# andreaskoepf/faster-rcnn.torch

Hardware: AMD Instinct MI355X
Metric: images/sec (vgg_small 800x450 fwd+bwd) (higher is better)
Workload: dtype f32 (conv / Linear(13824,1024) operands as 2 x fp16 split planes: 22 significand bits, 3 MFMA partial products; fp32 accumulate)

## Files before the change

faster-rcnn.torch_amd/_lib.py:

```python
import ctypes as C
import os

_HERE = os.path.dirname(os.path.abspath(__file__))
SO_PATH = os.environ.get("FRCNN_LIB_PATH") or os.path.join(_HERE, "libfrcnn_hip.so")

KC_NAMES = ["conv_igemm_k3", "conv_igemm_other", "conv_wgrad_k3", "conv_wgrad_other", "gemm", "elemwise",
            "roi", "rpn", "nms", "optim", "image", "conv_x3", "conv_wgradx"]


class FrcnnError(RuntimeError):
    pass


class ModelDesc(C.Structure):
    _fields_ = [
        ("nblocks", C.c_int),
        ("filters", C.c_int * 8), ("ksize", C.c_int * 8), ("pad", C.c_int * 8), ("conv_steps", C.c_int * 8),
        ("dropout", C.c_float * 8),
        ("nheads", C.c_int),
        ("head_k", C.c_int * 8), ("head_n", C.c_int * 8), ("head_input", C.c_int * 8),
        ("ncls", C.c_int),
        ("cls_n", C.c_int * 8), ("cls_bn", C.c_int * 8),
        ("cls_dropout", C.c_float * 8),
        ("class_count", C.c_int),
        ("kh", C.c_int), ("kw", C.c_int),
    ]


vp = C.c_void_p
_SIGS = {
    "frcnn_version": ([], C.c_int),
    "frcnn_set_option": ([C.c_char_p, C.c_int], C.c_int),
    "frcnn_get_option": ([C.c_char_p, C.POINTER(C.c_int)], C.c_int),
    "frcnn_last_error": ([], C.c_char_p),
    "frcnn_device_count": ([C.POINTER(C.c_int)], C.c_int),
    "frcnn_set_device": ([C.c_int], C.c_int),
    "frcnn_device_name": ([C.c_char_p, C.c_int], C.c_int),
    "frcnn_malloc": ([C.POINTER(vp), C.c_size_t], C.c_int),
    "frcnn_free": ([vp], C.c_int),
    "frcnn_host_alloc": ([C.POINTER(vp), C.c_size_t], C.c_int),
    "frcnn_host_free": ([vp], C.c_int),
    "frcnn_memcpy_h2d": ([vp, vp, C.c_size_t, vp], C.c_int),
    "frcnn_memcpy_d2h": ([vp, vp, C.c_size_t, vp], C.c_int),
    "frcnn_memcpy_d2d": ([vp, vp, C.c_size_t, vp], C.c_int),
    "frcnn_stream_sync": ([vp], C.c_int),
    "frcnn_zero": ([vp, C.c_size_t, vp], C.c_int),
    "frcnn_scale": ([vp, C.c_longlong, C.c_float, vp], C.c_int),
    "frcnn_add": ([vp, vp, C.c_longlong, vp], C.c_int),
    "frcnn_prof_enable": ([C.c_int], C.c_int),
    "frcnn_prof_collect": ([vp, vp, vp, vp], C.c_int),
    "frcnn_nms_workspace_bytes": ([C.c_int], C.c_size_t),
    "frcnn_nms_device": ([vp, C.c_int, C.c_int, C.c_float, C.c_int, C.c_int, vp, vp, vp, C.c_size_t, vp], C.c_int),
    "frcnn_nms_device_classes": ([vp, C.c_int, C.c_int, C.c_float, C.c_int, C.c_int, vp, vp, vp, vp, C.c_size_t, vp], C.c_int),
    "frcnn_nms_device_n": ([vp, C.c_int, vp, C.c_int, C.c_float, C.c_int, C.c_int, vp, vp, vp, vp, C.c_size_t, vp], C.c_int),
    "frcnn_roi_windows": ([vp, vp, C.c_int, vp, C.c_int, C.c_int, C.c_int, vp, vp], C.c_int),
    "frcnn_detect_post": ([vp, vp, vp, vp, vp, C.c_int, C.c_int, C.c_double, vp, vp, vp, vp, vp, vp], C.c_int),
    "frcnn_detect_gather": ([vp, vp, C.c_int, vp, vp, vp, vp, vp, vp, vp, vp, vp, vp], C.c_int),
    "frcnn_nms_host": ([vp, C.c_int, C.c_int, C.c_float, C.c_int, C.c_int, vp, vp], C.c_int),
    "frcnn_conv2d_forward": ([vp, C.c_int, C.c_int, C.c_int, vp, vp, vp, vp, C.c_int, C.c_int, C.c_int, vp, vp], C.c_int),
    "frcnn_conv2d_backward_input": ([vp, C.c_int, C.c_int, C.c_int, vp, C.c_int, C.c_int, C.c_int, vp, C.c_int, vp], C.c_int),
    "frcnn_conv2d_backward_weight": ([vp, C.c_int, C.c_int, C.c_int, vp, vp, vp, C.c_int, C.c_int, C.c_int, vp, vp, vp], C.c_int),
    "frcnn_maxpool_act_forward": ([vp, C.c_int, C.c_int, C.c_int, vp, vp, vp, vp, vp], C.c_int),
    "frcnn_maxpool_act_backward": ([vp, vp, vp, C.c_int, C.c_int, C.c_int, vp, vp, vp, vp, vp, vp], C.c_int),
    "frcnn_act_forward": ([vp, C.c_int, C.c_longlong, vp, vp, vp, vp], C.c_int),
    "frcnn_act_backward": ([vp, vp, C.c_int, C.c_longlong, vp, vp, vp, vp, vp, vp], C.c_int),
    "frcnn_roi_pool_forward": ([vp, C.c_int, C.c_int, C.c_int, vp, C.c_int, C.c_int, C.c_int, vp, vp, vp], C.c_int),
    "frcnn_roi_pool_backward": ([vp, C.c_int, C.c_int, C.c_int, vp, vp, C.c_int, C.c_int, C.c_int, vp], C.c_int),
    "frcnn_rpn_scan_workspace_bytes": ([vp, vp], C.c_size_t),
    "frcnn_rpn_scan": ([vp, vp, vp, vp, vp, C.c_double, C.c_double, C.c_double, C.c_int, vp, vp, vp, vp, vp, vp, C.c_size_t, vp], C.c_int),
    "frcnn_rpn_loss": ([vp, vp, vp, vp, vp, vp, vp, vp, C.c_int, C.c_int, C.c_int, vp, vp, vp, vp], C.c_int),
    "frcnn_loss_accumulate": ([vp, C.c_int, vp, vp], C.c_int),
    "frcnn_linear_forward": ([vp, C.c_int, C.c_int, vp, vp, C.c_int, vp, vp], C.c_int),
    "frcnn_linear_backward": ([vp, vp, C.c_int, C.c_int, vp, C.c_int, vp, vp, vp, vp], C.c_int),
    "frcnn_rmsprop": ([vp, vp, vp, C.c_longlong, C.c_float, C.c_float, C.c_float, vp], C.c_int),
    "frcnn_scale_rmsprop": ([vp, vp, C.c_float, vp, C.c_longlong, C.c_float, C.c_float, C.c_float, vp], C.c_int),
    "frcnn_scale_rmsprop_dev": ([vp, vp, vp, vp, C.c_longlong, C.c_float, C.c_float, C.c_float, vp], C.c_int),
    "frcnn_scale_rmsprop_slice": ([vp, vp, C.c_float, vp, C.c_longlong, C.c_longlong, C.c_float, C.c_float, C.c_float, vp], C.c_int),
    "frcnn_model_update_stream": ([vp, C.POINTER(vp)], C.c_int),
    "frcnn_model_update_fork": ([vp, vp], C.c_int),
    "frcnn_model_update_join": ([vp, vp], C.c_int),
    "frcnn_pnet_wait_backward_begun": ([vp, vp], C.c_int),
    "frcnn_pnet_wait_heads_done": ([vp, vp], C.c_int),
    "frcnn_pnet_wait_block_done": ([vp, C.c_int, vp], C.c_int),
    "frcnn_pnet_refresh_packs": ([vp, vp, C.c_int, vp], C.c_int),
    "frcnn_pnet_invalidate_packs": ([vp], C.c_int),
    "frcnn_model_create": ([C.POINTER(ModelDesc), C.POINTER(vp)], C.c_int),
    "frcnn_model_destroy": ([vp], C.c_int),
    "frcnn_model_param_count": ([vp, C.POINTER(C.c_longlong), C.POINTER(C.c_longlong)], C.c_int),
    "frcnn_model_param_table": ([vp, vp, C.c_int, C.POINTER(C.c_int)], C.c_int),
    "frcnn_model_localizer_layers": ([vp, C.c_int, vp, C.c_int, C.POINTER(C.c_int)], C.c_int),
    "frcnn_model_debug_buffer": ([vp, C.c_int, C.c_int, C.POINTER(vp), C.POINTER(C.c_longlong)], C.c_int),
    "frcnn_pnet_forward": ([vp, vp, vp, C.c_int, C.c_int, C.c_int, vp, C.c_ulonglong, vp], C.c_int),
    "frcnn_pnet_forward_async_heads": ([vp, vp, vp, C.c_int, C.c_int, vp, C.c_ulonglong, vp], C.c_int),
    "frcnn_pnet_output": ([vp, C.c_int, C.POINTER(vp), C.POINTER(C.c_int), C.POINTER(C.c_int), C.POINTER(C.c_int)], C.c_int),
    "frcnn_pnet_delta": ([vp, C.c_int, C.POINTER(vp)], C.c_int),
    "frcnn_pnet_set_sparse_deltas": ([vp, C.c_int, vp, C.c_int], C.c_int),
    "frcnn_pnet_zero_deltas": ([vp, vp], C.c_int),
    "frcnn_pnet_backward_heads_begin": ([vp, vp, vp, vp], C.c_int),
    "frcnn_pnet_anchor_loss_begin": ([vp, vp, vp, vp, vp, vp, vp, C.c_int, C.c_int, C.c_int, vp, vp, vp, vp, vp], C.c_int),
    "frcnn_pnet_anchor_loss_wait": ([vp, vp], C.c_int),
    "frcnn_pnet_backward_heads_join": ([vp, vp, C.POINTER(C.c_int)], C.c_int),
    "frcnn_pnet_backward": ([vp, vp, vp, vp], C.c_int),
    "frcnn_pnet_wait_block_gradients": ([vp, C.c_int, vp], C.c_int),
    "frcnn_cnet_forward": ([vp, vp, vp, C.c_int, C.c_int, vp, C.c_ulonglong, vp, vp, vp, vp], C.c_int),
    "frcnn_cnet_backward": ([vp, vp, vp, vp, vp, vp, vp], C.c_int),
    "frcnn_cnet_backward_join": ([vp, vp], C.c_int),
    "frcnn_cnet_losses": ([vp, vp, vp, vp, C.c_int, C.c_int, C.c_int, vp, vp, vp, vp], C.c_int),
    "frcnn_cnet_decode": ([vp, C.c_int, C.c_int, vp, vp, vp], C.c_int),
    "frcnn_anchors_create": ([vp, vp, vp, vp, C.c_int, C.c_int, C.POINTER(vp)], C.c_int),
    "frcnn_anchors_destroy": ([vp], C.c_int),
    "frcnn_anchors_assemble": ([vp, vp, C.c_int, C.c_double, C.c_double, C.c_double, C.c_double, C.c_int, C.c_int, C.c_int, vp,
                               C.POINTER(C.c_int), vp, vp, C.c_int, C.POINTER(C.c_int), C.POINTER(C.c_int)], C.c_int),
    "frcnn_comm_get_unique_id": ([vp], C.c_int),
    "frcnn_comm_exchange_id_file": ([C.c_char_p, C.c_int, vp, C.c_int], C.c_int),
    "frcnn_comm_init_rank": ([C.POINTER(vp), C.c_int, C.c_int, vp], C.c_int),
    "frcnn_comm_init_rank_timeout": ([C.POINTER(vp), C.c_int, C.c_int, vp, C.c_int], C.c_int),
    "frcnn_comm_init_rank_file": ([C.POINTER(vp), C.c_int, C.c_int, C.c_char_p, C.c_int], C.c_int),
    "frcnn_comm_destroy": ([vp], C.c_int),
    "frcnn_comm_info": ([vp, C.POINTER(C.c_int), C.POINTER(C.c_int)], C.c_int),
    "frcnn_comm_query": ([vp, C.POINTER(C.c_int), C.POINTER(C.c_int), C.POINTER(C.c_int)], C.c_int),
    "frcnn_allreduce_f32": ([vp, vp, C.c_longlong, vp], C.c_int),
    "frcnn_allreduce_f64": ([vp, vp, C.c_longlong, vp], C.c_int),
    "frcnn_broadcast_f32": ([vp, vp, C.c_longlong, C.c_int, vp], C.c_int),
    "frcnn_image_rgb2yuv": ([vp, vp, C.c_int, C.c_int, vp], C.c_int),
    "frcnn_image_rgb2hsv": ([vp, vp, C.c_int, C.c_int, vp], C.c_int),
    "frcnn_image_rgb2lab": ([vp, vp, C.c_int, C.c_int, vp], C.c_int),
    "frcnn_image_scale": ([vp, C.c_int, C.c_int, C.c_int, vp, C.c_int, C.c_int, vp, C.c_int, vp], C.c_int),
    "frcnn_image_scale_u8": ([vp, C.c_int, C.c_int, vp, C.c_int, C.c_int, vp, C.c_int, vp], C.c_int),
    "frcnn_image_crop_flip": ([vp, C.c_int, C.c_int, C.c_int, C.c_int, C.c_int, C.c_int, C.c_int, C.c_int, C.c_int, vp, vp], C.c_int),
    "frcnn_image_normalize_workspace_bytes": ([C.c_int], C.c_size_t),
    "frcnn_image_normalize": ([vp, C.c_int, C.c_int, C.c_int, C.c_int, C.c_int, vp, C.c_size_t, vp], C.c_int),
    "frcnn_image_contrastive_norm": ([vp, C.c_int, C.c_int, vp, C.c_int, C.c_float, vp, vp, vp], C.c_int),
}

_lib = None


def exported_symbols():
    return sorted(_SIGS.keys())


def load():
    global _lib
    if _lib is not None:
        return _lib
    if not os.path.exists(SO_PATH):
        raise FrcnnError(
            "libfrcnn_hip.so not found at %s -- build it with `python -c 'import __graft_entry__ as g; g.build()'` "
            "(there is no CPU fallback for the product path)" % SO_PATH)
    try:
        import torch
    except ImportError:
        pass
    L = C.CDLL(SO_PATH)
    for name, (args, res) in _SIGS.items():
        fn = getattr(L, name)
        fn.argtypes = args
        fn.restype = res
    _lib = L
    return L


def check(rc):
    if rc != 0:
        raise FrcnnError("libfrcnn_hip: %s (code %d)" % (load().frcnn_last_error().decode("utf-8", "replace"), rc))


def call(name, *args):
    check(getattr(load(), name)(*args))
```

faster-rcnn.torch_amd/csrc/api.cpp:

```cpp
#include <cmath>
#include <cstring>
#include <vector>
#include <mutex>

#include "kernels.h"

namespace frcnn {

static thread_local std::string g_err;

void set_error(const char* fmt, ...) {
  char buf[1024];
  va_list ap;
  va_start(ap, fmt);
  vsnprintf(buf, sizeof(buf), fmt, ap);
  va_end(ap);
  g_err = buf;
}

struct ProfRec { int klass; double flops, bytes; hipEvent_t a, b; hipStream_t s; };
static hipEvent_t g_prof_base = nullptr;
static unsigned g_prof_mask = 0;
static std::vector<ProfRec> g_recs;
static std::vector<hipEvent_t> g_pool;
// ... 92 lines not shown
    if (!g_prof_base) FR_HIP(hipEventCreate(&g_prof_base));
    FR_HIP(hipDeviceSynchronize());
    FR_HIP(hipEventRecord(g_prof_base, nullptr));
  }
  g_prof_mask = (unsigned)class_mask;
  return FRCNN_OK;
}
int frcnn_prof_collect(long long* launches, double* ms, double* flops, double* bytes) {
  FR_HIP(hipDeviceSynchronize());
  for (int k = 0; k < KC_COUNT; ++k) { launches[k] = 0; ms[k] = 0; flops[k] = 0; bytes[k] = 0; }
  FILE* dump = (getenv("FRCNN_PROF_DUMP") && g_prof_base) ? fopen(getenv("FRCNN_PROF_DUMP"), "a") : nullptr;
  for (auto& r : g_recs) {
    float t = 0.f;
    FR_HIP(hipEventElapsedTime(&t, r.a, r.b));
    if (dump) {
      float t0 = 0.f;
      if (hipEventElapsedTime(&t0, g_prof_base, r.a) == hipSuccess)
        fprintf(dump, "%d %p %.1f %.1f\n", r.klass, (void*)r.s, t0 * 1e3, t * 1e3);
    }
    launches[r.klass] += 1; ms[r.klass] += t; flops[r.klass] += r.flops; bytes[r.klass] += r.bytes;
    g_pool.push_back(r.a);
    g_pool.push_back(r.b);
  }
  if (dump) { fprintf(dump, "-1 0 0 0\n"); fclose(dump); }
  g_recs.clear();
  return FRCNN_OK;
}

size_t frcnn_nms_workspace_bytes(int n) { return nms_workspace_bytes(n); }
int frcnn_nms_device(const float* boxes, int n, int ncols, float overlap, int key_mode, int key_col,
                     long long* pick, int* count, void* ws, size_t ws_bytes, void* stream) {
  return nms_device(boxes, n, ncols, overlap, key_mode, key_col, pick, count, ws, ws_bytes, S(stream));
}
int frcnn_nms_device_classes(const float* boxes, int n, int ncols, float overlap, int key_mode, int key_col, const int* cls,
                             long long* pick, int* count, void* ws, size_t ws_bytes, void* stream) {
  return nms_device(boxes, n, ncols, overlap, key_mode, key_col, pick, count, ws, ws_bytes, S(stream), cls);
}
int frcnn_nms_device_n(const float* boxes, int n_cap, const int* n_dev, int ncols, float overlap, int key_mode, int key_col,
                       const int* cls, long long* pick, int* count, void* ws, size_t ws_bytes, void* stream) {
  FR_CHECK(n_dev, "frcnn_nms_device_n: NULL device count");
  return nms_device(boxes, n_cap, ncols, overlap, key_mode, key_col, pick, count, ws, ws_bytes, S(stream), cls, n_dev);
}
int frcnn_roi_windows(const double* rect, const long long* pick, int k, const int* layers_host, int nlayers, int fmH, int fmW,
                      int* wins, void* stream) {
  FR_CHECK(rect && wins && (layers_host || nlayers == 0), "frcnn_roi_windows: NULL argument");
  return roi_windows(rect, pick, k, layers_host, nlayers, fmH, fmW, wins, S(stream));
}
int frcnn_detect_post(const int* cls, const float* conf, const float* bbox, const double* rect, const long long* pick, int R,
                      int bgclass, double min_conf, float* bb, int* kc, int* keep_row, double* r2, int* K_dev, void* stream) {
  return detect_post(cls, conf, bbox, rect, pick, R, bgclass, min_conf, bb, kc, keep_row, r2, K_dev, S(stream));
}
int frcnn_detect_gather(const long long* wpick, const int* nwin_dev, int cap, const int* keep_row, const int* kc, const float* bb,
                        const double* r2, const long long* pick, const float* match_p, const double* match_rect,
                        const int* match_idx, double* rec, void* stream) {
  return detect_gather(wpick, nwin_dev, cap, keep_row, kc, bb, r2, pick, match_p, match_rect, match_idx, rec, S(stream));
}
int frcnn_nms_host(const float* boxes_host, int n, int ncols, float overlap, int key_mode, int key_col,
                   long long* pick_host, int* count_host) {
  if (n <= 0) { *count_host = 0; return FRCNN_OK; }
  size_t wsb = nms_workspace_bytes(n);
  char* buf = nullptr;
  size_t bb = ((size_t)n * ncols * 4 + 255) / 256 * 256, pb = ((size_t)n * 8 + 255) / 256 * 256;
  FR_HIP(hipMalloc((void**)&buf, bb + pb + 256 + wsb));
  float* dboxes = (float*)buf;
  long long* dpick = (long long*)(buf + bb);
  int* dcount = (int*)(buf + bb + pb);
  void* ws = buf + bb + pb + 256;
  int rc = FRCNN_OK;
  hipError_t e = hipMemcpy(dboxes, boxes_host, (size_t)n * ncols * 4, hipMemcpyHostToDevice);
  if (e == hipSuccess) rc = nms_device(dboxes, n, ncols, overlap, key_mode, key_col, dpick, dcount, ws, wsb, 0);
  if (e == hipSuccess && rc == FRCNN_OK) e = hipMemcpy(count_host, dcount, 4, hipMemcpyDeviceToHost);
  if (e == hipSuccess && rc == FRCNN_OK && *count_host > 0)
    e = hipMemcpy(pick_host, dpick, (size_t)*count_host * 8, hipMemcpyDeviceToHost);
  (void)hipFree(buf);
  if (e != hipSuccess) { set_error("frcnn_nms_host: %s", hipGetErrorString(e)); return FRCNN_ERR_HIP; }
  return rc;
}

#define X3_REC_BYTES ((size_t)(2 * AMAX_REC + 4) * 4)
static int x3_f16_records(float** out) {
  *out = nullptr;
  if (!get_x3_f16()) return FRCNN_OK;
  FR_HIP(hipMalloc((void**)out, X3_REC_BYTES));
  return FRCNN_OK;
}

static int scale_fits_f16_form(const float* in_scale, int C, hipStream_t s, bool* ok) {
  *ok = true;
  if (!in_scale) return FRCNN_OK;
  std::vector<float> h((size_t)C);
  FR_HIP(hipMemcpyAsync(h.data(), in_scale, (size_t)C * 4, hipMemcpyDeviceToHost, s));
  FR_HIP(hipStreamSynchronize(s));
  for (float v : h) if (!(std::fabs(v) <= 1.f)) { *ok = false; break; }
  return FRCNN_OK;
}

int frcnn_conv2d_forward(const float* in, int C, int H, int W, const float* in_slope, const float* in_scale,
                         const float* weight, const float* bias, int O, int k, int pad, float* out,
                         void* stream) {
  float* wf = nullptr;
  if (conv_x3_eligible(C, O, k) && (k == 3 || (!in_slope && !in_scale))) {
    FR_HIP(hipMalloc((void**)&wf, conv_x3_pack_bytes(C, O, k)));
    float* am = nullptr;
    bool unit = true;
    int rcx = scale_fits_f16_form(in_scale, C, S(stream), &unit);
    if (rcx == FRCNN_OK && unit) rcx = x3_f16_records(&am);
    float* const amw = am ? am + AMAX_REC : nullptr;
    float* const aws = am ? am + 2 * AMAX_REC : nullptr;
    if (am && rcx == FRCNN_OK) {
      rcx = tensor_absmax(in, (long)C * H * W, am, S(stream));
      if (rcx == FRCNN_OK) rcx = tensor_absmax(weight, (long)O * C * k * k, amw, S(stream));
    }
    if (rcx == FRCNN_OK) rcx = conv_x3_pack(weight, O, C, k, 0, wf, S(stream), H + 2 * pad - k + 1, W + 2 * pad - k + 1, amw, aws);
    if (rcx == FRCNN_OK) rcx = conv_x3(in, C, H, W, in_slope, in_scale, wf, bias, O, k, pad, out, OUT_STORE, 0, S(stream), 0, nullptr, am, aws);
    (void)hipStreamSynchronize(S(stream));
    (void)hipFree(wf); (void)hipFree(am);
    return rcx;
  }
  FR_HIP(hipMalloc((void**)&wf, conv_pack_floats(C, O, k) * 4));
  int rc = conv_pack_weights(weight, O, C, k, wf, nullptr, S(stream));
  if (rc == FRCNN_OK) rc = conv_igemm(in, C, H, W, in_slope, in_scale, wf, bias, O, k, pad, out, OUT_STORE, 0, S(stream));
  (void)hipStreamSynchronize(S(stream));
  (void)hipFree(wf);
  return rc;
}
int frcnn_conv2d_backward_input(const float* gout, int O, int Ho, int Wo, const float* weight, int C, int k,
                                int pad, float* gin, int accumulate, void* stream) {
  float* wd = nullptr;
  if (conv_x3_eligible(O, C, k)) {
    FR_HIP(hipMalloc((void**)&wd, conv_x3_pack_bytes(O, C, k)));
    float* am = nullptr;
    int rcx = x3_f16_records(&am);
    float* const amw = am ? am + AMAX_REC : nullptr;
    float* const aws = am ? am + 2 * AMAX_REC : nullptr;
    if (am && rcx == FRCNN_OK) {
      rcx = tensor_absmax(gout, (long)O * Ho * Wo, am, S(stream));
      if (rcx == FRCNN_OK) rcx = tensor_absmax(weight, (long)O * C * k * k, amw, S(stream));
    }
    if (rcx == FRCNN_OK) rcx = conv_x3_pack(weight, O, C, k, 1, wd, S(stream), Ho + 2 * (k - 1 - pad) - k + 1, Wo + 2 * (k - 1 - pad) - k + 1, amw, aws);
    if (rcx == FRCNN_OK) rcx = conv_x3(gout, O, Ho, Wo, nullptr, nullptr, wd, nullptr, C, k, k - 1 - pad, gin, accumulate ? OUT_ADD : OUT_STORE, 0, S(stream), 0, nullptr, am, aws);
    (void)hipStreamSynchronize(S(stream));
    (void)hipFree(wd); (void)hipFree(am);
    return rcx;
  }
  FR_HIP(hipMalloc((void**)&wd, conv_pack_floats(O, C, k) * 4));
  int rc = conv_pack_weights(weight, O, C, k, nullptr, wd, S(stream));
  if (rc == FRCNN_OK)
    rc = conv_igemm(gout, O, Ho, Wo, nullptr, nullptr, wd, nullptr, C, k, k - 1 - pad, gin,
                    accumulate ? OUT_ADD : OUT_STORE, 0, S(stream));
  (void)hipStreamSynchronize(S(stream));
  (void)hipFree(wd);
  return rc;
}
int frcnn_conv2d_backward_weight(const float* in, int C, int H, int W, const float* in_slope,
                                 const float* in_scale, const float* gout, int O, int k, int pad,
                                 float* gweight, float* gbias, void* stream) {
  size_t wsb = conv_wgrad_workspace_bytes(C, H, W, O, k, pad);
  void* ws = nullptr;
  FR_HIP(hipMalloc(&ws, wsb));
  int rc = FRCNN_OK;
  float* am = nullptr;
  bool unit = true;
  rc = scale_fits_f16_form(in_scale, C, S(stream), &unit);
  if (rc == FRCNN_OK && unit && k == 3 && conv_wgradx_eligible(C, O, k)) rc = x3_f16_records(&am);
  if (am && rc == FRCNN_OK) {
    rc = tensor_absmax(in, (long)C * H * W, am, S(stream));
    if (rc == FRCNN_OK) rc = tensor_absmax(gout, (long)O * (H + 2 * pad - k + 1) * (W + 2 * pad - k + 1), am + AMAX_REC, S(stream));
  }
  if (rc == FRCNN_OK)
    rc = conv_wgrad(in, C, H, W, in_slope, in_scale, gout, O, k, pad, gweight, ws, wsb, S(stream), nullptr, am, am ? am + AMAX_REC : nullptr);
  (void)hipStreamSynchronize(S(stream));
  (void)hipFree(ws); (void)hipFree(am);
  FR_TRY(rc);
  if (gbias) {
    int Ho = H + 2 * pad - k + 1, Wo = W + 2 * pad - k + 1;
    FR_TRY(channel_sum(gout, O, (long)Ho * Wo, gbias, S(stream)));
  }
  return FRCNN_OK;
}

int frcnn_maxpool_act_forward(const float* x, int C, int H, int W, const float* slope, const float* scale,
                              float* out, unsigned char* idx, void* stream) {
  return maxpool_act_forward(x, C, H, W, slope, scale, out, idx, S(stream));
}
int frcnn_maxpool_act_backward(const float* gpool, const unsigned char* idx, const float* x, int C, int H, int W,
                               const float* slope, const float* scale, float* gx, float* gbias, float* gslope,
                               void* stream) {
  return maxpool_act_backward(gpool, idx, x, C, H, W, slope, scale, gx, gbias, gslope, S(stream));
}
int frcnn_act_forward(const float* x, int C, long long hw, const float* slope, const float* scale, float* y,
                      void* stream) {
  return act_forward(x, C, hw, slope, scale, y, S(stream));
}
int frcnn_act_backward(const float* gy, const float* x, int C, long long hw, const float* slope,
                       const float* scale, float* gx, float* gbias, float* gslope, void* stream) {
  return act_backward(gy, x, C, hw, slope, scale, gx, gbias, gslope, S(stream));
}

int frcnn_roi_pool_forward(const float* fmap, int C, int H, int W, const int* wins, int R, int kh, int kw,
                           float* out, int* idx, void* stream) {
  return roi_pool_forward(fmap, C, H, W, wins, R, kh, kw, out, idx, S(stream));
}
int frcnn_roi_pool_backward(float* gmap, int C, int H, int W, const float* gout, const int* idx, int R, int kh,
                            int kw, void* stream) {
  return roi_pool_backward(gmap, C, H, W, gout, idx, R, kh, kw, S(stream));
}

static void to_layers(const float* const* maps, const int* H, const int* W, RpnLayers* L) {
  for (int l = 0; l < 4; ++l) { L->map[l] = maps ? maps[l] : nullptr; L->H[l] = H[l]; L->W[l] = W[l]; }
}
size_t frcnn_rpn_scan_workspace_bytes(const int* H, const int* W) {
  RpnLayers L;
  to_layers(nullptr, H, W, &L);
  return rpn_scan_workspace_bytes(L);
}
int frcnn_rpn_scan(const float* const* maps, const int* H, const int* W, const float* anchor_w,
                   const float* anchor_h, double img_w, double img_h, double p_threshold, int cap,
                   float* match_p, int* match_idx, double* match_rect, float* match_box, int* count,
                   void* ws, size_t ws_bytes, void* stream) {
  RpnLayers L;
  to_layers(maps, H, W, &L);
  return rpn_scan(L, anchor_w, anchor_h, img_w, img_h, p_threshold, cap, match_p, match_idx, match_rect,
                  match_box, count, ws, ws_bytes, S(stream));
}
int frcnn_rpn_loss(const float* const* maps, float* const* deltas, const int* H, const int* W, const int* ex_idx,
                   const double* ex_anchor, const double* ex_roi, const int* ex_class, int npos, int nneg,
                   int bgclass, double* ex_loss, float* crtarget, float* cctarget, void* stream) {
  RpnLayers L;
  to_layers(maps, H, W, &L);
  return rpn_loss(L, deltas, ex_idx, ex_anchor, ex_roi, ex_class, npos, nneg, bgclass, ex_loss, crtarget,
                  cctarget, S(stream));
}

int frcnn_loss_accumulate(const double* ex_loss, int E, double* acc, void* stream) {
  return loss_accumulate(ex_loss, E, acc, S(stream));
}

int frcnn_linear_forward(const float* x, int R, int I, const float* weight, const float* bias, int O, float* y,
                         void* stream) {
  if (linear_x_eligible(1, R, I, O)) {
    void* xp = nullptr;
    FR_HIP(hipMalloc(&xp, (size_t)3 * R * I * 2));
    float* am = nullptr;
    int rc = x3_f16_records(&am);
    if (am && rc == FRCNN_OK) {
      rc = tensor_absmax(x, (long)R * I, am, S(stream));
      if (rc == FRCNN_OK) rc = tensor_absmax(weight, (long)O * I, am + AMAX_REC, S(stream));
    }
    if (rc == FRCNN_OK) rc = split_planes(x, R, I, xp, nullptr, S(stream), am);
    if (rc == FRCNN_OK) rc = linear_x_forward(xp, R, I, weight, bias, O, y, S(stream), 0, nullptr, am, am ? am + AMAX_REC : nullptr);
    (void)hipStreamSynchronize(S(stream));
    (void)hipFree(xp); (void)hipFree(am);
    return rc;
  }
  return gemm_f32(x, I, 1, weight, 1, I, y, O, R, O, I, OUT_STORE, bias, S(stream));
}
int frcnn_linear_backward(const float* x, const float* gy, int R, int I, const float* weight, int O, float* gx,
                          float* gweight, float* gbias, void* stream) {
  const bool xd = gx && linear_x_eligible(2, R, I, O), xw = gweight && linear_x_eligible(4, R, I, O);
  if (xd || xw) {
    const size_t Rp = (size_t)linear_x_rows_padded(R);
    void *gp = nullptr, *gpT = nullptr, *xpT = nullptr;
    int rc = FRCNN_OK;
    auto alloc = [&](void** p, size_t bytes) {
      if (rc != FRCNN_OK) return;
      hipError_t e = hipMalloc(p, bytes);
      if (e != hipSuccess) { set_error("frcnn_linear_backward: hipMalloc(%zu) failed: %s", bytes, hipGetErrorString(e)); rc = FRCNN_ERR_HIP; }
    };
    if (xd) alloc(&gp, (size_t)3 * R * O * 2);
    if (xw) { alloc(&gpT, (size_t)3 * O * Rp * 2); alloc(&xpT, (size_t)3 * I * Rp * 2); }
    float* am = nullptr;
    if (rc == FRCNN_OK && xd) rc = x3_f16_records(&am);
    if (rc == FRCNN_OK && am) {
      rc = tensor_absmax(gy, (long)R * O, am, S(stream));
      if (rc == FRCNN_OK) rc = tensor_absmax(weight, (long)O * I, am + AMAX_REC, S(stream));
      if (rc == FRCNN_OK) rc = split_planes(gy, R, O, gp, nullptr, S(stream), am);
      if (rc == FRCNN_OK && gpT) rc = split_planes(gy, R, O, nullptr, gpT, S(stream));
    } else if (rc == FRCNN_OK) rc = split_planes(gy, R, O, gp, gpT, S(stream));
    if (rc == FRCNN_OK && xw) rc = split_planes(x, R, I, nullptr, xpT, S(stream));
    if (rc == FRCNN_OK && xd) rc = linear_x_dgrad(gp, R, O, weight, I, gx, OUT_STORE, S(stream), 0, nullptr, am, am ? am + AMAX_REC : nullptr);
    if (rc == FRCNN_OK && xw) rc = linear_x_wgrad(gpT, xpT, R, O, I, gweight, S(stream));
    (void)hipStreamSynchronize(S(stream));
    (void)hipFree(gp); (void)hipFree(gpT); (void)hipFree(xpT); (void)hipFree(am);
    FR_TRY(rc);
    if (gx && !xd) FR_TRY(gemm_f32(gy, O, 1, weight, I, 1, gx, I, R, I, O, OUT_STORE, nullptr, S(stream)));
    if (gweight && !xw) FR_TRY(gemm_f32(gy, 1, O, x, I, 1, gweight, I, O, I, R, OUT_ADD, nullptr, S(stream)));
    if (gbias) FR_TRY(channel_sum_cols(gy, R, O, gbias, S(stream)));
    return FRCNN_OK;
  }
  if (gx) FR_TRY(gemm_f32(gy, O, 1, weight, I, 1, gx, I, R, I, O, OUT_STORE, nullptr, S(stream)));
  if (gweight) FR_TRY(gemm_f32(gy, 1, O, x, I, 1, gweight, I, O, I, R, OUT_ADD, nullptr, S(stream)));
  if (gbias) FR_TRY(channel_sum_cols(gy, R, O, gbias, S(stream)));
  return FRCNN_OK;
}

int frcnn_rmsprop(float* x, const float* g, float* m, long long n, float lr, float alpha, float eps,
                  void* stream) {
  return rmsprop_step(x, const_cast<float*>(g), m, n, lr, alpha, eps, 1.f, false, S(stream));
}

int frcnn_scale_rmsprop(float* x, float* g, float gscale, float* m, long long n, float lr, float alpha, float eps,
                        void* stream) {
  return rmsprop_step(x, g, m, n, lr, alpha, eps, gscale, true, S(stream));
}
int frcnn_scale_rmsprop_slice(float* x, float* g, float gscale, float* m, long long lo, long long hi, float lr, float alpha,
                              float eps, void* stream) {
  return rmsprop_slice(x, g, m, lo, hi, lr, alpha, eps, gscale, gscale != 1.0f, S(stream));
}
int frcnn_scale_rmsprop_dev(float* x, float* g, const double* gcount_dev, float* m, long long n, float lr, float alpha,
                            float eps, void* stream) {
  FR_CHECK(gcount_dev, "frcnn_scale_rmsprop_dev: NULL divisor");
  return rmsprop_step(x, g, m, n, lr, alpha, eps, 1.f, true, S(stream), gcount_dev);
}

int frcnn_cnet_losses(float* crout, const float* crtarget, const float* ccout, const float* cctarget, int R,
                      int npos, int ncls, float* crdelta, float* ccdelta, double* loss2, void* stream) {
  return cnet_losses(crout, crtarget, ccout, cctarget, R, npos, ncls, crdelta, ccdelta, loss2, S(stream));
}
int frcnn_cnet_decode(const float* cls_out, int R, int ncls, int* cls, float* conf, void* stream) {
  return cnet_decode(cls_out, R, ncls, cls, conf, S(stream));
}

int frcnn_image_rgb2yuv(const float* rgb, float* yuv, int H, int W, void* stream) {
  FR_CHECK(rgb != yuv, "image_rgb2yuv: in-place conversion is not supported");
  return image_rgb2yuv(rgb, yuv, H, W, S(stream));
}
int frcnn_image_rgb2hsv(const float* rgb, float* hsv, int H, int W, void* stream) {
  FR_CHECK(rgb != hsv, "image_rgb2hsv: in-place conversion is not supported");
  return image_rgb2hsv(rgb, hsv, H, W, S(stream));
}
int frcnn_image_rgb2lab(const float* rgb, float* lab, int H, int W, void* stream) {
// ... 27 lines not shown
```

faster-rcnn.torch_amd/csrc/conv.hip:

```cpp
#include <cstdlib>

#include "kernels.h"
#include "amax.h"
#include <type_traits>

namespace frcnn {

typedef float f32x16 __attribute__((ext_vector_type(16)));

int conv_cc(int k) { return k == 1 ? 32 : (k == 3 ? 8 : 2); }
int conv_mpad(int M) { return M <= 64 ? 64 : cdiv(M, 128) * 128; }
size_t conv_pack_floats(int Kchan, int M, int k) {
  int cc = conv_cc(k);
  return (size_t)cdiv(Kchan, cc) * cc * k * k * conv_mpad(M);
}

__global__ void pack_weights_kernel(const float* __restrict__ w, int O, int C, int k, int mode,
                                    int Kchan_pad, int M, int Mpad, float* __restrict__ dst) {
  long total = (long)Kchan_pad * k * k * Mpad;
  for (long t = (long)blockIdx.x * blockDim.x + threadIdx.x; t < total;
       t += (long)gridDim.x * blockDim.x) {
    int m = (int)(t % Mpad);
    long row = t / Mpad;
    int h = (int)(row & 1);
// ... 1095 lines not shown
  a.kyGroups = k / tys;
  long base = (long)a.oTiles * a.cTiles * a.kyGroups;
  long npix = (long)a.tilesX * a.tilesY;
  a.nSplit = (int)std::max<long>(1, std::min<long>(npix, (512 + base / 2) / base));
  a.dbg = 0;
  if (const char* e = getenv("FRCNN_WG_DBG")) a.dbg = atoi(e);
  if (const char* e = getenv("FRCNN_WG_NSPLIT")) a.nSplit = (int)std::max<long>(1, std::min<long>(npix, atoi(e)));
}

__global__ __launch_bounds__(256) void wgrad_reduce4_kernel(const float* __restrict__ slab, int nSplit, int taps, int OC,
                                                            float* __restrict__ gw) {
  __shared__ float4 sh[4][64];
  const long total = (long)taps * OC;
  const int tx = threadIdx.x & 63, g = threadIdx.x >> 6;
  for (long t0 = (long)blockIdx.x * 256; t0 < total; t0 += (long)gridDim.x * 256) {
    const long t = t0 + 4 * tx;
    float4 a0 = {0.f, 0.f, 0.f, 0.f}, a1 = a0, a2 = a0, a3 = a0;
    auto add = [](float4& a, const float4 x) { a.x += x.x; a.y += x.y; a.z += x.z; a.w += x.w; };
    if (t < total) {
      int s = g;
      for (; s + 12 < nSplit; s += 16) {
        const float4 x0 = *reinterpret_cast<const float4*>(slab + (size_t)s * total + t);
        const float4 x1 = *reinterpret_cast<const float4*>(slab + (size_t)(s + 4) * total + t);
        const float4 x2 = *reinterpret_cast<const float4*>(slab + (size_t)(s + 8) * total + t);
        const float4 x3 = *reinterpret_cast<const float4*>(slab + (size_t)(s + 12) * total + t);
        add(a0, x0); add(a1, x1); add(a2, x2); add(a3, x3);
      }
      for (; s < nSplit; s += 4) add(a0, *reinterpret_cast<const float4*>(slab + (size_t)s * total + t));
    }
    sh[g][tx] = make_float4((a0.x + a1.x) + (a2.x + a3.x), (a0.y + a1.y) + (a2.y + a3.y), (a0.z + a1.z) + (a2.z + a3.z),
                            (a0.w + a1.w) + (a2.w + a3.w));
    __syncthreads();
    if (g == 0 && t < total) {
      const int tap = (int)(t / OC);
      const int oc = (int)(t - (long)tap * OC);
      const float4 p0 = sh[0][tx], p1 = sh[1][tx], p2 = sh[2][tx], p3 = sh[3][tx];
      float* d = gw + (size_t)oc * taps + tap;
      d[0] += (p0.x + p1.x) + (p2.x + p3.x);
      d[taps] += (p0.y + p1.y) + (p2.y + p3.y);
      d[2 * (size_t)taps] += (p0.z + p1.z) + (p2.z + p3.z);
      d[3 * (size_t)taps] += (p0.w + p1.w) + (p2.w + p3.w);
    }
    __syncthreads();
  }
}

int wgrad_reduce(const float* slab, int nSplit, int taps, int OC, float* gw, hipStream_t s) {
  const long total = (long)taps * OC;
  if (OC % 4 == 0 && ((uintptr_t)slab & 15) == 0) {
    const int rgrid = (int)std::min<long>(cdivl(total, 256), 4096);
    hipLaunchKernelGGL(wgrad_reduce4_kernel, dim3(rgrid), dim3(256), 0, s, slab, nSplit, taps, OC, gw);
    return FRCNN_OK;
  }
  const int rgrid = (int)std::min<long>(cdivl(total, 64), 4096);
  hipLaunchKernelGGL(wgrad_reduce_kernel, dim3(rgrid), dim3(256), 0, s, slab, nSplit, taps, OC, gw);
  return FRCNN_OK;
}

__global__ __launch_bounds__(256) void wgrad_reduce_map_kernel(const float* __restrict__ slab, int nSplit, int taps, int O, int C,
                                                               float* __restrict__ gw, WgradMap map) {
  __shared__ float4 sh[4][64];
  const long OC = (long)O * C, total = (long)taps * OC;
  const int tx = threadIdx.x & 63, g = threadIdx.x >> 6;
  for (long t0 = (long)blockIdx.x * 256; t0 < total; t0 += (long)gridDim.x * 256) {
    const long t = t0 + 4 * tx;
    float4 a0 = {0.f, 0.f, 0.f, 0.f}, a1 = a0, a2 = a0, a3 = a0;
    auto add = [](float4& a, const float4 x) { a.x += x.x; a.y += x.y; a.z += x.z; a.w += x.w; };
    if (t < total) {
      int s = g;
      for (; s + 12 < nSplit; s += 16) {
        const float4 x0 = *reinterpret_cast<const float4*>(slab + (size_t)s * total + t);
        const float4 x1 = *reinterpret_cast<const float4*>(slab + (size_t)(s + 4) * total + t);
        const float4 x2 = *reinterpret_cast<const float4*>(slab + (size_t)(s + 8) * total + t);
        const float4 x3 = *reinterpret_cast<const float4*>(slab + (size_t)(s + 12) * total + t);
        add(a0, x0); add(a1, x1); add(a2, x2); add(a3, x3);
      }
      for (; s < nSplit; s += 4) add(a0, *reinterpret_cast<const float4*>(slab + (size_t)s * total + t));
    }
    sh[g][tx] = make_float4((a0.x + a1.x) + (a2.x + a3.x), (a0.y + a1.y) + (a2.y + a3.y), (a0.z + a1.z) + (a2.z + a3.z),
                            (a0.w + a1.w) + (a2.w + a3.w));
    __syncthreads();
    if (g == 0 && t < total) {
      const int tap = (int)(t / OC);
      const long oc = t - (long)tap * OC;
      const int o = (int)(oc / C), c = (int)(oc - (long)o * C);
      const int od = map.omap ? map.omap[o] : o;
      const float4 p0 = sh[0][tx], p1 = sh[1][tx], p2 = sh[2][tx], p3 = sh[3][tx];
      const float r[4] = {(p0.x + p1.x) + (p2.x + p3.x), (p0.y + p1.y) + (p2.y + p3.y), (p0.z + p1.z) + (p2.z + p3.z),
                          (p0.w + p1.w) + (p2.w + p3.w)};
      if (od >= 0) {
#pragma unroll
        for (int e = 0; e < 4; ++e) {
          const int cd = map.cmap ? map.cmap[c + e] : c + e;
          if (cd >= 0) gw[((size_t)od * map.Cfull + cd) * taps + tap] += r[e];
        }
      }
    }
    __syncthreads();
  }
}
int wgrad_reduce_map(const float* slab, int nSplit, int taps, int O, int C, float* gw, const WgradMap& map, hipStream_t s) {
  FR_CHECK(map.Cfull > 0 && C % 4 == 0 && ((uintptr_t)slab & 15) == 0, "wgrad_reduce_map: the full tensor's channel count is missing, or C %% 4 != 0");
  const int rgrid = (int)std::min<long>(cdivl((long)taps * O * C, 256), 4096);
  hipLaunchKernelGGL(wgrad_reduce_map_kernel, dim3(rgrid), dim3(256), 0, s, slab, nSplit, taps, O, C, gw, map);
  return FRCNN_OK;
}

size_t conv_wgrad_workspace_bytes(int Cin, int H, int W, int O, int k, int pad) {
  if (k == 3 && Cin % 64 == 0 && O % 64 == 0) {
    WgradArgs b;
    b.Cin = Cin; b.H = H; b.W = W; b.O = O; b.pad = pad; b.Ho = H + 2 * pad - k + 1; b.Wo = W + 2 * pad - k + 1;
    wgrad_plan(b, k);
    return std::max((size_t)b.nSplit * k * k * O * Cin * 4 + 256, conv_wgradx_workspace_bytes(Cin, H, W, O, pad));
  }
  WgradArgs a;
  a.Cin = Cin; a.H = H; a.W = W; a.O = O; a.pad = pad;
  a.Ho = H + 2 * pad - k + 1; a.Wo = W + 2 * pad - k + 1;
  wgrad_plan(a, k);
  return (size_t)a.nSplit * (k * k * O * Cin + O + 1) * 4 + 256;
}

template <int KS, int TYS, int PM>
static int launch_wgrad_pm(WgradArgs& a, int klass, double flops, float* gw, hipStream_t s) {
  size_t lds = ((size_t)64 * WG_NTP + (size_t)64 * (PM == 2 ? 129 : WG_PP)) * 4;
  static bool attr_set = false;
  if (!attr_set) {
    FR_HIP(hipFuncSetAttribute(reinterpret_cast<const void*>(conv_wgrad_kernel<KS, TYS, PM>),
                               hipFuncAttributeMaxDynamicSharedMemorySize, 160 * 1024));
    attr_set = true;
  }
  int grid = a.oTiles * a.cTiles * a.kyGroups * a.nSplit;
  double bytes = 4.0 * ((double)a.Cin * a.H * a.W + (double)a.O * a.Ho * a.Wo);
  if (frcnn::prof_enabled(klass)) frcnn::prof_before(klass, s);
  hipLaunchKernelGGL((conv_wgrad_kernel<KS, TYS, PM>), dim3(grid), dim3(256), lds, s, a);
  const int OC = a.O * a.Cin;
  long total = (long)KS * KS * OC;
  int rgrid = (int)std::min<long>(cdivl(total, 64), 4096);
  if (!(a.dbg & 1))
    hipLaunchKernelGGL(wgrad_reduce_kernel, dim3(rgrid), dim3(256), 0, s, (const float*)a.slab, a.nSplit, KS * KS, OC, gw);
  if (frcnn::prof_enabled(klass)) frcnn::prof_after(klass, flops, bytes, s);
  FR_LAUNCH_CHECK();
  return FRCNN_OK;
}

template <int KS, int TYS>
static int launch_wgrad(WgradArgs& a, int klass, double flops, float* gw, hipStream_t s) {
  const int pplane = (a.TH + TYS - 1) * (a.TW + KS - 1);
  if (pplane <= 128) return launch_wgrad_pm<KS, TYS, 2>(a, klass, flops, gw, s);
  return launch_wgrad_pm<KS, TYS, 3>(a, klass, flops, gw, s);
}

int conv_wgrad(const float* in, int Cin, int H, int W, const float* in_slope, const float* in_scale,
               const float* g, int O, int k, int pad, float* gw, void* ws, size_t ws_bytes, hipStream_t s, float* gbias,
               const float* amax_in, const float* amax_g, const WgradMap* map) {
  WgradArgs a;
  a.in = in; a.in_slope = in_slope; a.in_scale = in_scale; a.g = g;
  a.Cin = Cin; a.H = H; a.W = W; a.O = O; a.pad = pad;
  a.Ho = H + 2 * pad - k + 1; a.Wo = W + 2 * pad - k + 1;
  FR_CHECK(k == 1 || k == 3 || k == 5 || k == 7, "conv_wgrad: unsupported kernel size %d", k);
  if (conv_wgradx_eligible(Cin, O, k)) return conv_wgradx(in, Cin, H, W, in_slope, in_scale, g, O, pad, gw, ws, ws_bytes, s, gbias, amax_in, amax_g, map);
  FR_CHECK(!map || (!map->omap && !map->cmap), "conv_wgrad: a gathered weight gradient needs a conv_wgradx shape");
  if (gbias) FR_TRY(channel_sum(g, O, (long)a.Ho * a.Wo, gbias, s));
  FR_CHECK((long)Cin * H * W < (1L << 31) && (long)O * a.Ho * a.Wo < (1L << 31), "conv_wgrad: tensor too large for 32-bit offsets");
  g_wgrad_first_ok = (in_slope == nullptr && in_scale == nullptr);
  wgrad_plan(a, k);
  size_t need = (size_t)a.nSplit * k * k * O * Cin * 4 + 256;
  FR_CHECK(ws && ws_bytes >= need, "conv_wgrad: workspace too small (%zu < %zu)", ws_bytes, need);
  a.slab = (float*)(((uintptr_t)ws + 255) / 256 * 256);
  double flops = 2.0 * O * Cin * k * k * (double)a.Ho * a.Wo;
  int klass = k == 3 ? KC_CONV_WGRAD_K3 : KC_CONV_WGRAD_OTHER;
  if (wgrad_is_first(Cin, O, k, a.Wo)) {
    FR_CHECK((double)O * a.Ho * a.Wo * 4.0 < 4294967295.0 && (double)Cin * H * W * 4.0 < 4294967295.0,
             "conv_wgrad: first-layer tensors too large for 32-bit buffer resources");
    size_t lds = ((size_t)64 * W1_GP + W1_PATCH) * 4;
    static bool attr_set = false;
    if (!attr_set) {
      FR_HIP(hipFuncSetAttribute(reinterpret_cast<const void*>(conv_wgrad_first_kernel<3, false>),
                                 hipFuncAttributeMaxDynamicSharedMemorySize, 160 * 1024));
      attr_set = true;
    }
    if (frcnn::prof_enabled(klass)) frcnn::prof_before(klass, s);
    hipLaunchKernelGGL((conv_wgrad_first_kernel<3, false>), dim3(a.nSplit), dim3(256), lds, s, a, WgradFirstFused{});
    wgrad_reduce_first(a.slab, a.nSplit, O * Cin, gw, s);
    if (frcnn::prof_enabled(klass)) frcnn::prof_after(klass, flops, 4.0 * ((double)Cin * H * W + (double)O * a.Ho * a.Wo), s);
    FR_LAUNCH_CHECK();
    return FRCNN_OK;
  }
  if (k == 3) return launch_wgrad<3, 3>(a, klass, flops, gw, s);
  if (k == 1) return launch_wgrad<1, 1>(a, klass, flops, gw, s);
  if (k == 5) return launch_wgrad<5, 1>(a, klass, flops, gw, s);
  return launch_wgrad<7, 1>(a, klass, flops, gw, s);
}

bool conv_wgrad_first_pooled_eligible(int Cin, int O, int k, int Wo) { return k == 3 && Cin * 9 < 32 && O <= 64 && Wo >= 2; }
int conv_wgrad_first_pooled(const float* in, int Cin, int H, int W, const float* gpool, const unsigned char* pidx, const float* x,
                            const float* slope, int O, int pad, float* gw, float* gbias, float* gslope, void* ws, size_t ws_bytes,
                            hipStream_t s) {
  FR_CHECK(conv_wgrad_first_pooled_eligible(Cin, O, 3, W + 2 * pad - 2) && slope, "conv_wgrad_first_pooled: not a first-layer shape");
  FR_CHECK((double)O * (H + 2 * pad - 2) * (W + 2 * pad - 2) * 4.0 < 4294967295.0 && (double)Cin * H * W * 4.0 < 4294967295.0,
           "conv_wgrad_first_pooled: tensors too large for 32-bit buffer resources");
  WgradArgs a;
  a.in = in; a.in_slope = nullptr; a.in_scale = nullptr; a.g = nullptr;
  a.Cin = Cin; a.H = H; a.W = W; a.O = O; a.pad = pad;
  a.Ho = H + 2 * pad - 2; a.Wo = W + 2 * pad - 2;
  a.TH = W1_TH; a.TW = W1_TW;
  a.tilesX = cdiv(a.Wo, W1_TW); a.tilesY = cdiv(a.Ho, W1_TH);
  a.oTiles = a.cTiles = a.kyGroups = 1;
  a.nSplit = std::min(512, a.tilesX * a.tilesY);
  a.dbg = 0;
  if (const char* e = getenv("FRCNN_WG_DBG")) a.dbg = atoi(e);
  const size_t need = (size_t)a.nSplit * (9 * O * Cin + O + 1) * 4 + 256;
  FR_CHECK(ws && ws_bytes >= need, "conv_wgrad_first_pooled: workspace too small (%zu < %zu)", ws_bytes, need);
  a.slab = (float*)(((uintptr_t)ws + 255) / 256 * 256);
  WgradFirstFused q{gpool, pidx, x, slope, gslope, gbias, (a.Ho - 2 + 1) / 2 + 1, (a.Wo - 2 + 1) / 2 + 1};
  const size_t lds = ((size_t)64 * W1_GP + W1_PATCH + W1_TW) * 4;
  static bool attr_set = false;
  if (!attr_set) {
    FR_HIP(hipFuncSetAttribute(reinterpret_cast<const void*>(conv_wgrad_first_kernel<3, true>),
                               hipFuncAttributeMaxDynamicSharedMemorySize, 160 * 1024));
    attr_set = true;
  }
  const double flops = 2.0 * O * Cin * 9 * (double)a.Ho * a.Wo;
  if (frcnn::prof_enabled(KC_CONV_WGRAD_K3)) frcnn::prof_before(KC_CONV_WGRAD_K3, s);
  hipLaunchKernelGGL((conv_wgrad_first_kernel<3, true>), dim3(a.nSplit), dim3(256), lds, s, a, q);
  wgrad_reduce_first(a.slab, a.nSplit, O * Cin, gw, s, O + 1, gbias, gslope);
  if (frcnn::prof_enabled(KC_CONV_WGRAD_K3))
    frcnn::prof_after(KC_CONV_WGRAD_K3, flops, 4.0 * ((double)Cin * H * W + (double)O * a.Ho * a.Wo * 1.3125), s);
  FR_LAUNCH_CHECK();
  return FRCNN_OK;
}

}
```

faster-rcnn.torch_amd/csrc/kernels.h:

```cpp
#pragma once
#include <algorithm>

#include "common.h"

namespace frcnn {

int conv_cc(int k);
int conv_mpad(int M);
size_t conv_pack_floats(int Kchan, int M, int k);
int conv_pack_weights(const float* w, int O, int C, int k, float* wf, float* wd, hipStream_t s);
struct PackJob { long w_off; long total; float* dst; int O, C, k, mode, Mpad, blk_begin, nblk; };
PackJob conv_pack_job(long w_off, int O, int C, int k, int mode, float* dst);
int conv_pack_assign_blocks(PackJob* jobs, int njobs, int total_blocks);
int conv_pack_weights_multi(const float* weights, const PackJob* jobs_dev, int njobs, int grid, hipStream_t s);

enum { OUT_STORE = 0, OUT_ADD = 1 };
struct IgemmPool { float* out; unsigned char* idx; const float* slope; const float* scale; float* amax = nullptr; };
int conv_igemm(const float* in, int Cin, int H, int W, const float* in_slope, const float* in_scale,
               const float* wp, const float* bias, int M, int k, int pad, float* out, int out_mode,
               double algo_flops, hipStream_t s, int ws_slot = 0,
               const IgemmPool* pool = nullptr, bool* pool_fused = nullptr);

void set_split_bf16(int on);
int get_split_bf16();
bool conv_x3_eligible(int Cin, int M, int k);
size_t conv_x3_pack_bytes(int Kchan, int M, int k);
struct PackXJob {
  long w_off; long total; void* dst; const float* amax; float* amax_w; int O, C, k, mode, bm, blk_begin, nblk;
  const int* oidx = nullptr; const int* cidx = nullptr; int Cs = 0; long bias_off = 0; float* bias_dst = nullptr;
};
PackXJob conv_x3_pack_job(long w_off, int O, int C, int k, int mode, void* dst, int Ho, int Wo);
int conv_x3_pack_assign_blocks(PackXJob* jobs, int njobs);
int conv_x3_pack_multi(const float* weights, const PackXJob* jobs_dev, int njobs, int grid, hipStream_t s);
int conv_x3_pack(const float* w, int O, int C, int k, int mode, void* dst, hipStream_t s, int Ho, int Wo,
                 const float* amax_rec_w = nullptr, float* amax_w = nullptr);
#define AMAX_REC 16400
#define AMAX_MAX_BLOCKS 16384
int tensor_absmax(const float* x, long n, float* rec, hipStream_t s);
struct AmaxJob { long off; long n; float* out; int blk_begin; };
int tensor_absmax_assign_blocks(AmaxJob* jobs, int njobs);
long tensor_absmax_record_floats(long n);
int tensor_absmax_multi(const float* w, const AmaxJob* jobs_dev, int njobs, int grid, hipStream_t s);
void set_x3_f16(int on);
int get_x3_f16();
int conv_x3(const float* in, int Cin, int H, int W, const float* in_slope, const float* in_scale, const void* wp,
            const float* bias, int M, int k, int pad, float* out, int out_mode, double algo_flops, hipStream_t s, int ws_slot = 0,
            const struct X3PostAct* post = nullptr, const float* amax_in = nullptr, const float* amax_w = nullptr,
            float* amax_out = nullptr);
struct X3PostAct {
  const float* x;
  const float* slope;
  const float* scale;
  float* gslope;
};

bool conv_wgradx_eligible(int Cin, int O, int k);
size_t conv_wgradx_workspace_bytes(int Cin, int H, int W, int O, int pad);
struct WgradMap { const int* omap = nullptr; const int* cmap = nullptr; int Cfull = 0; };
int conv_wgradx(const float* in, int Cin, int H, int W, const float* in_slope, const float* in_scale, const float* g, int O,
                int pad, float* gw, void* ws, size_t ws_bytes, hipStream_t s, float* gbias = nullptr,
                const float* amax_in = nullptr, const float* amax_g = nullptr,
                const WgradMap* map = nullptr);
int wgrad_reduce(const float* slab, int nSplit, int taps, int OC, float* gw, hipStream_t s);
int wgrad_reduce_map(const float* slab, int nSplit, int taps, int O, int C, float* gw, const WgradMap& map, hipStream_t s);
bool conv_wgrad_first_pooled_eligible(int Cin, int O, int k, int Wo);
int conv_wgrad_first_pooled(const float* in, int Cin, int H, int W, const float* gpool, const unsigned char* pidx, const float* x,
                            const float* slope, int O, int pad, float* gw, float* gbias, float* gslope, void* ws, size_t ws_bytes,
                            hipStream_t s);

size_t conv_wgrad_workspace_bytes(int Cin, int H, int W, int O, int k, int pad);
int conv_wgrad(const float* in, int Cin, int H, int W, const float* in_slope, const float* in_scale,
               const float* g, int O, int k, int pad, float* gw, void* ws, size_t ws_bytes, hipStream_t s,
               float* gbias = nullptr,
               const float* amax_in = nullptr, const float* amax_g = nullptr,
               const WgradMap* map = nullptr);

bool deterministic();
void set_deterministic(bool on);
int det_workspace(hipStream_t s, size_t floats, float** out);

int fill_zero(void* p, size_t bytes, hipStream_t s);
int scale_inplace(float* x, long n, float sc, hipStream_t s);
int add_inplace(float* y, const float* x, long n, hipStream_t s);
int act_forward(const float* x, int C, long hw, const float* slope, const float* scale, float* y,
                hipStream_t s);
int maxpool_act_forward(const float* x, int C, int H, int W, const float* slope, const float* scale,
                        float* out, unsigned char* idx, hipStream_t s, float* amax = nullptr);
int maxpool_act_backward(const float* gpool, const unsigned char* idx, const float* x, int C, int H,
                         int W, const float* slope, const float* scale, float* gx, float* gbias,
                         float* gslope, hipStream_t s, float* amax = nullptr);
int act_backward(const float* gy, const float* x, int C, long hw, const float* slope,
                 const float* scale, float* gx, float* gbias, float* gslope, hipStream_t s, float* amax = nullptr);
int channel_sum(const float* g, int C, long hw, float* gbias, hipStream_t s);
int channel_sum_cols(const float* g, int R, int O, float* gb, hipStream_t s);
int gather_positions(const float* src, int C, long hw, const int* pos, int P, float* dst, const float* slope,
                     float* dst_act, hipStream_t s);
int im2col_positions(const float* X, int C, int H, int W, int k, int Wo, const int* pos, int P, float* col, hipStream_t s);
int col2im_positions_add(const float* col, int C, int H, int W, int k, int Wo, const int* pos, int P, float* gX,
                         hipStream_t s);
int dropout_channel_mask(float* scale, int C, float p, unsigned long long seed, hipStream_t s);
int fill_value(float* x, long n, float v, hipStream_t s);
int rmsprop_step(float* x, float* g, float* m, long n, float lr, float alpha, float eps, float gscale,
                 bool scale_first, hipStream_t s, const double* gcount_dev = nullptr);
int rmsprop_slice(float* x, float* g, float* m, long lo, long hi, float lr, float alpha, float eps, float gscale, bool scale_first,
                  hipStream_t s);

#define FRCNN_HEAD_OUT 18
struct HeadJob {
  int Cin, H, W, k, Ho, Wo, n;
  int P; const int* pos;
  const float* in; float* gin;
  const float *bias3, *slope, *bias1;
  float *gbias3, *gslope, *gbias1;
  float* out; const float* delta;
  float *COL, *HX, *HY, *OUT, *D, *GH, *DX;
  const float* hx_slab; int hx_splits;
};
struct HeadJobs { HeadJob j[4]; int n; };
int heads_im2col(const HeadJobs& g, hipStream_t s);
int heads_bias_act(const HeadJobs& g, hipStream_t s);
int heads_scatter(const HeadJobs& g, hipStream_t s);
int heads_gather_delta(const HeadJobs& g, hipStream_t s);
int heads_act_backward(const HeadJobs& g, hipStream_t s);
int heads_col2im(const HeadJobs& g, hipStream_t s);

struct GemmFold;
#define GEMM_GROUP_MAX 4
struct GemmJob {
  const float* A; long sAm, sAk; const float* B; long sBk, sBn; float* C; long ldc;
  int M, N, K, out_mode;
  int splits = 1;
  int kPerSplit = 0;
};
int gemm_f32_group(GemmJob* jobs, int n, hipStream_t s);
int gemm_f32(const float* A, long sAm, long sAk, const float* B, long sBk, long sBn, float* C,
             long ldc, int M, int N, int K, int out_mode, const float* bias_n, hipStream_t s, int ws_slot = 0,
             GemmFold* defer = nullptr);
int gemm_workspace_get(size_t need, float** out, int slot);
struct GemmFold {
  const float* slab = nullptr;
  int nSplit = 0;
  const float* bias = nullptr;
};
int gemm_reduce_slabs(const float* slab, int nSplit, int M, int N, const float* bias, float* C, long ldc, bool accumulate,
                      hipStream_t s);
void set_gemm_x_roles(int mask);
int get_gemm_x_roles();
bool linear_x_eligible(int role, int R, int I, int O);
int linear_x_rows_padded(int R);
int split_planes(const float* src, int R, int C, void* P , void* PT ,
                 hipStream_t s, const float* amax = nullptr);
int linear_x_forward(const void* Xp, int R, int I, const float* W, const float* bias, int O, float* y, hipStream_t s, int ws_slot = 0,
                     GemmFold* defer = nullptr, const float* amax_x = nullptr, const float* amax_w = nullptr);
int linear_x_dgrad(const void* Gp, int R, int O, const float* W, int I, float* gx, int out_mode, hipStream_t s, int ws_slot = 0,
                   GemmFold* defer = nullptr, const float* amax_g = nullptr, const float* amax_w = nullptr);
int linear_x_wgrad(const void* GpT, const void* XpT, int R, int O, int I, float* gw, hipStream_t s, int ws_slot = 0,
                   const float* amax_g = nullptr, const float* amax_x = nullptr);


int roi_pool_forward(const float* fmap, int C, int H, int W, const int* wins, int R, int kh, int kw,
                     float* out, int* idx, hipStream_t s);
int roi_pool_backward(float* gmap, int C, int H, int W, const float* gout, const int* idx, int R,
                      int kh, int kw, hipStream_t s);

struct RpnLayers {
  const float* map[4];
  int H[4], W[4];
};
int rpn_scan(const RpnLayers& L, const float* anchor_w, const float* anchor_h, double img_w,
             double img_h, double p_threshold, int cap, float* match_p, int* match_idx,
             double* match_rect, float* match_box, int* count, void* ws, size_t ws_bytes,
             hipStream_t s);
size_t rpn_scan_workspace_bytes(const RpnLayers& L);
int rpn_loss(const RpnLayers& L, float* const* delta, const int* ex_idx, const double* ex_anchor,
             const double* ex_roi, const int* ex_class, int npos, int nneg, int bgclass,
             double* ex_loss, float* crtarget, float* cctarget, hipStream_t s);

int loss_accumulate(const double* ex_loss, int E, double* acc, hipStream_t s);

size_t nms_workspace_bytes(int n);
int nms_device(const float* boxes, int n, int ncols, float overlap, int key_mode, int key_col,
               long long* pick, int* count, void* ws, size_t ws_bytes, hipStream_t s, const int* cls = nullptr,
               const int* n_dev = nullptr);
int roi_windows(const double* rect, const long long* pick, int k, const int* layers, int nlayers, int fmH, int fmW, int* wins,
                hipStream_t s);
int detect_post(const int* cls, const float* conf, const float* bbox, const double* rect, const long long* pick, int R,
                int bgclass, double min_conf, float* bb, int* kc, int* keep_row, double* r2, int* K_dev, hipStream_t s);
int detect_gather(const long long* wpick, const int* nwin_dev, int cap, const int* keep_row, const int* kc, const float* bb,
                  const double* r2, const long long* pick, const float* mp, const double* rect, const int* midx, double* rec,
                  hipStream_t s);

int bn_forward(const float* x, int R, int n, const float* gamma, const float* beta, float* running,
               int training, float* xhat, float* invstd, float* y, hipStream_t s);
int bn_backward(const float* gy, const float* xhat, const float* invstd, const float* gamma, int R,
                int n, int training, float* gx, float* ggamma, float* gbeta, hipStream_t s);
int prelu_dropout_forward(const float* x, long n, const float* slope, const float* mask, float inv_keep,
                          float* y, hipStream_t s);
int prelu_dropout_forward_gen(const float* x, long n, const float* slope, float* mask_out, float p,
                              unsigned long long seed, float* y, hipStream_t s);
int prelu_dropout_backward(const float* gy, const float* x, long n, const float* slope,
                           const float* mask, float inv_keep, float* gx, float* gslope, hipStream_t s);
int cnet_act_forward(const float* x, GemmFold src, int R, int n, const float* gamma, const float* beta, float* running,
                     int training, float* lin, float* xhat, float* invstd, float* pre, const float* slope, float* mask, bool gen,
                     float inv_keep, float p, unsigned long long seed, float* post, hipStream_t s);
int cnet_act_bn_backward(const float* gy, GemmFold src, const float* pre, const float* xhat, const float* invstd,
                         const float* gamma, const float* slope, const float* mask, float inv_keep, int R, int n, int training,
                         float* gx, float* ggamma, float* gbeta, float* gslope, hipStream_t s);
bool cnet_heads_fused_eligible(int nf, int nc);
int cnet_heads_forward(const float* x, int R, int nf, const float* Wb, const float* bb, const float* Wc, const float* bc, int nc,
                       float* bbox_out, float* logits, float* lsm, float* cls_out, hipStream_t s);
struct HeadsPostAct {
  const float* pre = nullptr;
  const float* mask = nullptr;
  float inv_keep = 1.f;
  const float* slope = nullptr;
  float* gslope = nullptr;
};
int cnet_heads_backward(const float* g_bbox, const float* g_cls, const float* lsm, int R, int nf, const float* Wb, const float* Wc,
                        int nc, float* glog, float* gfeat, hipStream_t s, const HeadsPostAct* post = nullptr);
int log_softmax_rows_fold(const float* x, GemmFold src, int R, int n, float* y, float* y2, hipStream_t s);
int dropout_mask(float* mask, long n, float p, unsigned long long seed, hipStream_t s);
struct DropoutJobs { float* ptr[8]; int C[8]; float p[8]; unsigned long long seed[8]; int n; };
int dropout_channel_masks(const DropoutJobs& j, hipStream_t s);
int log_softmax_rows(const float* x, int R, int n, float* y, hipStream_t s);
int cnet_losses(float* crout, const float* crtarget, const float* ccout, const float* cctarget, int R,
                int npos, int ncls, float* crdelta, float* ccdelta, double* loss2, hipStream_t s);
int log_softmax_backward(const float* gy, const float* lsm, int R, int n, float* gx, hipStream_t s);
int cnet_decode(const float* cls_lsm, int R, int ncls, int* cls_out, float* conf_out, hipStream_t s);
// ... 18 lines not shown
```

faster-rcnn.torch_amd/csrc/net.cpp:

```cpp
#include <array>
#include <vector>
#include <cmath>
#include <cstring>

#include "kernels.h"

namespace frcnn {

static const int HEAD_OUT = 18;
static const int SPARSE_MAX_POS = 512;

struct DevBuf {
  void* p = nullptr;
  size_t bytes = 0;
  bool owned = true;
  void view(void* ptr, size_t n) { p = ptr; bytes = n; owned = false; }
  int ensure(size_t need) {
    if (need <= bytes) return FRCNN_OK;
    if (p && owned) (void)hipFree(p);
    owned = true;
    p = nullptr; bytes = 0;
    FR_HIP(hipMalloc(&p, need + 64));
    bytes = need;
    return FRCNN_OK;
  }
  void release() { if (p && owned) (void)hipFree(p); p = nullptr; bytes = 0; owned = true; }
  float* f() const { return (float*)p; }
};

struct Conv {
  int Cin, Cout, k, pad;
  int H, W, Ho, Wo;
  long w_off, b_off, a_off;
  int block, step;
  DevBuf wf, wd;
  DevBuf wx, wxd;
  bool x_f = false, x_d = false;
  DevBuf x, gx;
  int am = -1;
};

struct Block {
  int first_conv, nconv;
  bool has_drop;
  float p_drop;
  DevBuf scale;
  DevBuf pooled, gpooled;
  DevBuf pidx;
  int Hp, Wp;
  int am = -1;
  bool dc_on = false;
  int nk = 0, nkM = 0, nkK = 0;
  const int* dc_idx = nullptr;
  DevBuf dc_bias;
};

struct Head {
  Conv c3;
  Conv c1;
  int input;
  DevBuf delta;
  const int* sp_pos = nullptr;
  int sp_count = -1;
  DevBuf spD, spHX, spHY, spGH, spCol, spDX;
  DevBuf spOut, spSlab;
  hipStream_t stream = nullptr;
  hipEvent_t done = nullptr;
  hipEvent_t gin_done = nullptr;
  bool gin_recorded = false;
};

struct ClsLayer {
  int in, n;
  bool bn;
  float p_drop;
  long w_off, b_off, bnw_off, bnb_off, a_off;
  DevBuf lin, pre, post, xhat, invstd, mask, g;
  DevBuf gin;
  DevBuf xp, xpT, gp, gpT;
  int x_form = 0;
  DevBuf am;
  const float* am_w_of = nullptr;
  long am_w_gen = -1;
};

}

using namespace frcnn;

static int g_drop_compact = -1;
static int drop_compact_on() {
  if (g_drop_compact < 0) g_drop_compact = getenv("FRCNN_DROP_COMPACT") ? (atoi(getenv("FRCNN_DROP_COMPACT")) != 0) : 1;
  return g_drop_compact;
}
static int pool_stream(int slot, hipStream_t* out) {
  static hipStream_t pool[8] = {};
  if (!pool[slot]) FR_HIP(hipStreamCreateWithFlags(&pool[slot], hipStreamNonBlocking));
  *out = pool[slot];
  return FRCNN_OK;
}

static int g_sparse_heads = -1;
static int sparse_heads_on() {
  if (g_sparse_heads < 0) g_sparse_heads = getenv("FRCNN_SPARSE_HEADS") ? (atoi(getenv("FRCNN_SPARSE_HEADS")) != 0) : 1;
  return g_sparse_heads;
}
static int g_static_weights = 0;
static long g_static_gen = 0;

struct frcnn_model {
  frcnn_model_desc d;
  std::vector<Conv> convs;
  std::vector<Block> blocks;
  std::vector<Head> heads;
  std::vector<ClsLayer> cls;
  long pnet_params = 0, total_params = 0;
  long bbox_w_off = 0, bbox_b_off = 0, clsw_off = 0, clsb_off = 0;
  int H = 0, W = 0;
  int training = 0;
  DevBuf delta_last;
  DevBuf zero_arena;
  size_t delta_bytes = 0, gpool_bytes = 0;
  DevBuf pack_jobs;
  DevBuf x3_jobs;
  DevBuf amax, amax_ws, amax_jobs;
  int n_amax = 0, n_amax_jobs = 0, amax_grid = 0;
  float* rec(int id) const { return (float*)amax.p + (size_t)id * AMAX_REC; }
  bool f16_packed = false;
  long eval_packs_gen = -1;
  const float* eval_packs_w = nullptr;
  int n_x3_all = 0, n_x3_fwd = 0, x3_grid_all = 0, x3_grid_fwd = 0;
  int n_pack_fwd = 0, n_pack_all = 0, n_pack_heads = 0, pack_grid_fwd = 0, pack_grid_all = 0, pack_grid_heads = 0;
  bool head_packs_fresh = false;
  struct PackGroup { int pk_off = 0, pk_n = 0, pk_grid = 0, am_off = 0, am_n = 0, am_grid = 0, x3_off = 0, x3_off16 = 0, x3_n = 0, x3_grid = 0; };
  std::vector<PackGroup> groups;
  unsigned fresh_mask = 0;
  const float* fresh_w = nullptr;
  bool fresh_f16 = false;
  static const int DC_RING = 4;
  char* dc_pin = nullptr; DevBuf dc_dev; size_t dc_slot_bytes = 0, dc_idx_off = 0; unsigned dc_step = 0;
  hipEvent_t dc_ev[DC_RING] = {};
  std::vector<PackXJob> x3_host, x3_host16;
  std::vector<int> x3_conv;
  DevBuf dbg_expand;
  std::vector<hipEvent_t> block_rd_ev;
  hipStream_t side = nullptr;
  hipStream_t cw = nullptr;
  hipEvent_t cw_fork = nullptr, cw_done = nullptr;
  bool cw_pending = false;
  std::vector<hipEvent_t> cw_ev;
  std::vector<hipEvent_t> fork_ev;
  hipEvent_t join_ev = nullptr;
  bool update_armed = false;
  hipEvent_t bwd_ev = nullptr;
  hipEvent_t upd_ev = nullptr, upd_join_ev = nullptr;
  bool head_x3_fresh = true;
  int am_bb_off = 0, am_bb_n = 0, am_bb_grid = 0;
  int pk_bb_off = 0, pk_bb_n = 0, pk_bb_grid = 0;
  bool heads_deferred = false;
  bool heads_sparse_fwd = false;
  const float* last_w = nullptr;
  hipEvent_t heads_gin_ev = nullptr;
  bool heads_gin = false;
  bool heads_begun = false;
  bool heads_joined = false;
  bool side_busy = false;
  hipEvent_t loss_ev = nullptr;
  hipEvent_t chain_ev = nullptr;
  std::vector<hipEvent_t> block_ev;
  bool block_ev_valid = false;
  bool loss_pending = false;
  DevBuf wg_ws;
  DevBuf wg_ws_first;
  DevBuf img;
  int R = 0, D = 0;
  const float* cnet_x = nullptr;
  DevBuf feat_g, logits, lsm, glog, gtmp;
  std::vector<std::array<long long, 4>> table;
};

static int pool_out(int n) { return (n - 2 + 1) / 2 + 1; }
static int refresh_group(frcnn_model* m, const float* w, int group, hipStream_t s);

static void build_layout(frcnn_model* m) {
  const frcnn_model_desc& d = m->d;
  long off = 0;
  int cin = 3;
  for (int b = 0; b < d.nblocks; ++b) {
    Block blk;
    blk.first_conv = (int)m->convs.size();
    blk.nconv = d.conv_steps[b];
    blk.has_drop = d.dropout[b] > 0.f;
    blk.p_drop = d.dropout[b];
    for (int s = 0; s < d.conv_steps[b]; ++s) {
      Conv c;
      c.Cin = cin; c.Cout = d.filters[b]; c.k = d.ksize[b]; c.pad = d.pad[b];
      c.block = b; c.step = s;
      long wsz = (long)c.Cout * c.Cin * c.k * c.k;
      c.w_off = off; c.b_off = off + wsz; c.a_off = off + wsz + c.Cout;
      m->table.push_back({c.w_off, wsz, 0, (long long)c.k * c.k * c.Cout});
      m->table.push_back({c.b_off, c.Cout, 1, 0});
      m->table.push_back({c.a_off, 1, 2, 0});
      off += wsz + c.Cout + 1;
      cin = c.Cout;
      m->convs.push_back(std::move(c));
    }
    m->blocks.push_back(std::move(blk));
  }
  for (int h = 0; h < d.nheads; ++h) {
    Head hd;
    hd.input = d.head_input[h] - 1;
    Conv& a = hd.c3;
    a.Cin = d.filters[hd.input]; a.Cout = d.head_n[h]; a.k = d.head_k[h]; a.pad = 0;
    a.block = -1; a.step = 0;
    long wsz = (long)a.Cout * a.Cin * a.k * a.k;
    a.w_off = off; a.b_off = off + wsz; a.a_off = off + wsz + a.Cout;
    m->table.push_back({a.w_off, wsz, 0, (long long)a.k * a.k * a.Cout});
    m->table.push_back({a.b_off, a.Cout, 1, 0});
    m->table.push_back({a.a_off, 1, 2, 0});
    off += wsz + a.Cout + 1;
    Conv& c = hd.c1;
    c.Cin = a.Cout; c.Cout = HEAD_OUT; c.k = 1; c.pad = 0; c.block = -1; c.step = 1;
    long w1 = (long)HEAD_OUT * c.Cin;
    c.w_off = off; c.b_off = off + w1; c.a_off = -1;
    m->table.push_back({c.w_off, w1, 0, (long long)HEAD_OUT});
    m->table.push_back({c.b_off, HEAD_OUT, 1, 0});
    off += w1 + HEAD_OUT;
    m->heads.push_back(std::move(hd));
  }
  m->pnet_params = off;
  int in = d.kh * d.kw * d.filters[d.nblocks - 1];
  m->D = in;
  for (int l = 0; l < d.ncls; ++l) {
    ClsLayer L;
    L.in = in; L.n = d.cls_n[l]; L.bn = d.cls_bn[l] != 0; L.p_drop = d.cls_dropout[l];
    L.w_off = off; L.b_off = off + (long)in * L.n;
    m->table.push_back({L.w_off, (long long)in * L.n, 3, in});
    m->table.push_back({L.b_off, L.n, 4, in});
    off += (long)in * L.n + L.n;
    L.bnw_off = L.bnb_off = -1;
    if (L.bn) {
      L.bnw_off = off; L.bnb_off = off + L.n;
      m->table.push_back({L.bnw_off, L.n, 5, 0});
      m->table.push_back({L.bnb_off, L.n, 6, 0});
      off += 2L * L.n;
    }
// ... 274 lines not shown
               desc->ncls >= 0 && desc->ncls <= 8,
           "frcnn_model_create: bad layer counts");
  for (int b = 0; b < desc->nblocks; ++b) {
    FR_CHECK(desc->ksize[b] == 1 || desc->ksize[b] == 3 || desc->ksize[b] == 5 || desc->ksize[b] == 7,
             "block %d: kernel size %d unsupported (1,3,5,7)", b + 1, desc->ksize[b]);
    FR_CHECK(desc->conv_steps[b] >= 1, "block %d: conv_steps must be >= 1", b + 1);
  }
  for (int h = 0; h < desc->nheads; ++h) {
    FR_CHECK(desc->head_input[h] >= 1 && desc->head_input[h] <= desc->nblocks, "anchor net %d: bad input", h + 1);
    FR_CHECK(desc->head_k[h] == 1 || desc->head_k[h] == 3 || desc->head_k[h] == 5 || desc->head_k[h] == 7,
             "anchor net %d: kernel size %d unsupported", h + 1, desc->head_k[h]);
  }
  frcnn_model* m = new frcnn_model();
  m->d = *desc;
  build_layout(m);
  *out = m;
  return FRCNN_OK;
}

int frcnn_model_destroy(frcnn_model* m) {
  if (!m) return FRCNN_OK;
  auto rel = [](Conv& c) { c.wf.release(); c.wd.release(); c.wx.release(); c.wxd.release(); c.x.release(); c.gx.release(); };
  for (auto& c : m->convs) rel(c);
  for (auto& b : m->blocks) { b.scale.release(); b.pooled.release(); b.gpooled.release(); b.pidx.release(); b.dc_bias.release(); }
  if (m->dc_pin) (void)hipHostFree(m->dc_pin);
  for (auto e : m->dc_ev) if (e) (void)hipEventDestroy(e);
  m->dc_dev.release(); m->dbg_expand.release();
  for (auto& h : m->heads) {
    rel(h.c3); rel(h.c1); h.delta.release(); h.spOut.release(); h.spSlab.release();
    h.spD.release(); h.spHX.release(); h.spHY.release(); h.spGH.release(); h.spCol.release(); h.spDX.release();
  }
  for (auto& l : m->cls) {
    l.lin.release(); l.pre.release(); l.post.release(); l.xhat.release(); l.invstd.release();
    l.mask.release(); l.g.release(); l.xp.release(); l.xpT.release(); l.gp.release(); l.gpT.release(); l.am.release();
  }
  m->img.release(); m->wg_ws.release(); m->wg_ws_first.release(); m->pack_jobs.release(); m->x3_jobs.release(); m->zero_arena.release(); m->amax.release(); m->amax_ws.release(); m->amax_jobs.release();
  for (auto e : m->fork_ev) (void)hipEventDestroy(e);
  for (auto& h : m->heads) {
    if (h.done) (void)hipEventDestroy(h.done);
    if (h.gin_done) (void)hipEventDestroy(h.gin_done);
  }
  if (m->chain_ev) (void)hipEventDestroy(m->chain_ev);
  if (m->join_ev) (void)hipEventDestroy(m->join_ev);
  if (m->bwd_ev) (void)hipEventDestroy(m->bwd_ev);
  if (m->heads_gin_ev) (void)hipEventDestroy(m->heads_gin_ev);
  if (m->upd_ev) (void)hipEventDestroy(m->upd_ev);
  if (m->upd_join_ev) (void)hipEventDestroy(m->upd_join_ev);
  for (auto e : m->block_rd_ev) (void)hipEventDestroy(e);
  for (auto e : m->cw_ev) (void)hipEventDestroy(e);
  if (m->cw_fork) (void)hipEventDestroy(m->cw_fork);
  if (m->cw_done) (void)hipEventDestroy(m->cw_done);
  if (m->loss_ev) (void)hipEventDestroy(m->loss_ev);
  for (auto e : m->block_ev) (void)hipEventDestroy(e);
  m->delta_last.release(); m->feat_g.release(); m->logits.release(); m->lsm.release(); m->glog.release();
  m->gtmp.release();
  delete m;
  return FRCNN_OK;
}

int frcnn_model_param_count(const frcnn_model* m, long long* total, long long* pnet) {
  if (total) *total = m->total_params;
  if (pnet) *pnet = m->pnet_params;
  return FRCNN_OK;
}

int frcnn_model_param_table(const frcnn_model* m, long long* table, int cap, int* n) {
  *n = (int)m->table.size();
  for (int i = 0; i < *n && i < cap; ++i)
    for (int j = 0; j < 4; ++j) table[4 * i + j] = m->table[i][j];
  return FRCNN_OK;
}

int frcnn_model_localizer_layers(const frcnn_model* m, int output_index, int* layers, int cap, int* n_out) {
  const frcnn_model_desc& d = m->d;
  FR_CHECK(output_index >= 1 && output_index <= d.nheads + 1, "localizer: output index %d out of range", output_index);
  int nb = output_index <= d.nheads ? d.head_input[output_index - 1] : d.nblocks;
  int n = 0;
  auto push = [&](int kW, int kH, int dW, int dH, int pW, int pH) {
    if (n < cap) { int* l = layers + 6 * n; l[0] = kW; l[1] = kH; l[2] = dW; l[3] = dH; l[4] = pW; l[5] = pH; }
    ++n;
  };
  for (int b = 0; b < nb; ++b) {
    for (int s = 0; s < d.conv_steps[b]; ++s) push(d.ksize[b], d.ksize[b], 1, 1, d.pad[b], d.pad[b]);
    push(2, 2, 2, 2, 0, 0);
  }
  if (output_index <= d.nheads) {
    int k = d.head_k[output_index - 1];
    push(k, k, 1, 1, 0, 0);
    push(1, 1, 1, 1, 0, 0);
  }
  *n_out = n;
  return FRCNN_OK;
}

static int g_side_stream = -1;
static bool side_enabled() {
  if (g_side_stream < 0) g_side_stream = !(getenv("FRCNN_SIDE_STREAM") && atoi(getenv("FRCNN_SIDE_STREAM")) == 0) ? 1 : 0;
  return g_side_stream != 0;
}

static int g_cnet_wgrad_async = getenv("FRCNN_CNET_WGRAD_ASYNC") ? (atoi(getenv("FRCNN_CNET_WGRAD_ASYNC")) != 0) : 1;

static int cw_join(frcnn_model* m, hipStream_t s) {
  if (m->cw_pending) {
    FR_HIP(hipStreamWaitEvent(s, m->cw_done, 0));
    m->cw_pending = false;
  }
  return FRCNN_OK;
}

int frcnn_cnet_backward_join(frcnn_model* m, void* stream) {
  FR_CHECK(m != nullptr, "cnet_backward_join: null model");
  return cw_join(m, S(stream));
}

static int ensure_update_stream(frcnn_model* m) {
  if (!m->cw) {
    FR_TRY(pool_stream(1, &m->cw));
    FR_HIP(hipEventCreateWithFlags(&m->cw_done, hipEventDisableTiming));
  }
  if (!m->upd_ev) FR_HIP(hipEventCreateWithFlags(&m->upd_ev, hipEventDisableTiming));
  if (!m->upd_join_ev) FR_HIP(hipEventCreateWithFlags(&m->upd_join_ev, hipEventDisableTiming));
  return FRCNN_OK;
}
int frcnn_model_update_stream(frcnn_model* m, void** stream) {
  FR_CHECK(m && stream, "model_update_stream: null argument");
  FR_TRY(ensure_update_stream(m));
  m->update_armed = true;
  *stream = (void*)m->cw;
  return FRCNN_OK;
}
int frcnn_model_update_fork(frcnn_model* m, void* stream) {
  FR_CHECK(m != nullptr, "model_update_fork: null model");
  FR_TRY(ensure_update_stream(m));
  FR_HIP(hipEventRecord(m->upd_ev, S(stream)));
  FR_HIP(hipStreamWaitEvent(m->cw, m->upd_ev, 0));
  return FRCNN_OK;
}
int frcnn_model_update_join(frcnn_model* m, void* stream) {
  FR_CHECK(m != nullptr, "model_update_join: null model");
  FR_TRY(ensure_update_stream(m));
  FR_HIP(hipEventRecord(m->upd_join_ev, m->cw));
  FR_HIP(hipStreamWaitEvent(S(stream), m->upd_join_ev, 0));
  return FRCNN_OK;
}

int frcnn_get_option(const char* name, int* value) {
  FR_CHECK(name != nullptr && value != nullptr, "get_option: null argument");
  if (strcmp(name, "side_stream") == 0) { *value = side_enabled() ? 1 : 0; return FRCNN_OK; }
  if (strcmp(name, "gemm_x_roles") == 0) { *value = get_gemm_x_roles(); return FRCNN_OK; }
  if (strcmp(name, "deterministic") == 0) { *value = deterministic() ? 1 : 0; return FRCNN_OK; }
  if (strcmp(name, "static_weights") == 0) { *value = g_static_weights; return FRCNN_OK; }
  if (strcmp(name, "drop_compact") == 0) { *value = drop_compact_on(); return FRCNN_OK; }
  if (strcmp(name, "sparse_heads") == 0) { *value = sparse_heads_on(); return FRCNN_OK; }
  if (strcmp(name, "winograd") == 0) { *value = 0; return FRCNN_OK; }
  if (strcmp(name, "cnet_wgrad_async") == 0) { *value = g_cnet_wgrad_async; return FRCNN_OK; }
  if (strcmp(name, "split_bf16") == 0) { *value = get_split_bf16(); return FRCNN_OK; }
  if (strcmp(name, "x3_f16") == 0) { *value = get_x3_f16(); return FRCNN_OK; }
  FR_CHECK(false, "get_option: unknown option '%s'", name);
  return FRCNN_OK;
}

int frcnn_set_option(const char* name, int value) {
  FR_CHECK(name != nullptr, "set_option: null name");
  if (strcmp(name, "side_stream") == 0) { g_side_stream = value ? 1 : 0; return FRCNN_OK; }
  if (strcmp(name, "deterministic") == 0) { set_deterministic(value != 0); return FRCNN_OK; }
  if (strcmp(name, "static_weights") == 0) { g_static_weights = value != 0; ++g_static_gen; return FRCNN_OK; }
  if (strcmp(name, "drop_compact") == 0) { g_drop_compact = value != 0; return FRCNN_OK; }
  if (strcmp(name, "sparse_heads") == 0) { g_sparse_heads = value != 0; return FRCNN_OK; }
  if (strcmp(name, "gemm_x_roles") == 0) { set_gemm_x_roles(value); return FRCNN_OK; }
  if (strcmp(name, "split_bf16") == 0) { set_split_bf16(value); return FRCNN_OK; }
  if (strcmp(name, "x3_f16") == 0) { set_x3_f16(value); return FRCNN_OK; }
  if (strcmp(name, "winograd") == 0) return FRCNN_OK;
  if (strcmp(name, "cnet_wgrad_async") == 0) { g_cnet_wgrad_async = value ? 1 : 0; return FRCNN_OK; }
  FR_CHECK(false, "set_option: unknown option '%s'", name);
  return FRCNN_OK;
}

static int ensure_head_streams(frcnn_model* m);
static int ensure_side(frcnn_model* m) {
  if (!m->side) {
    FR_TRY(pool_stream(0, &m->side));
    FR_HIP(hipEventCreateWithFlags(&m->join_ev, hipEventDisableTiming));
    FR_HIP(hipEventCreateWithFlags(&m->loss_ev, hipEventDisableTiming));
    FR_HIP(hipEventCreateWithFlags(&m->chain_ev, hipEventDisableTiming));
    for (auto& h : m->heads) FR_HIP(hipEventCreateWithFlags(&h.done, hipEventDisableTiming));
  }
  return FRCNN_OK;
}

static int ensure_head_streams(frcnn_model* m) {
  static const int head_streams = getenv("FRCNN_HEAD_STREAMS") ? atoi(getenv("FRCNN_HEAD_STREAMS")) : 1;
  size_t hi = 0;
  for (auto& h : m->heads) {
    if (head_streams && hi < 5 && !h.stream) FR_TRY(pool_stream(2 + (int)hi, &h.stream));
    ++hi;
  }
  return FRCNN_OK;
}

static hipStream_t head_stream(frcnn_model* m, size_t i) { return m->heads[i].stream ? m->heads[i].stream : m->side; }
static int head_slot(frcnn_model* m, size_t i) { return m->heads[i].stream ? 2 + (int)(i % 5) : 1; }

static int join_heads(frcnn_model* m, hipStream_t s) {
  for (auto& h : m->heads) {
    if (!h.stream) continue;
    FR_HIP(hipEventRecord(h.done, h.stream));
    FR_HIP(hipStreamWaitEvent(s, h.done, 0));
  }
  return FRCNN_OK;
}
static int join_side(frcnn_model* m, hipStream_t s) {
  if (!m->side || !m->side_busy) return FRCNN_OK;
  FR_TRY(join_heads(m, s));
  FR_HIP(hipEventRecord(m->join_ev, m->side));
  FR_HIP(hipStreamWaitEvent(s, m->join_ev, 0));
  m->side_busy = false;
  return FRCNN_OK;
}

static int chain(hipStream_t from, hipStream_t to, hipEvent_t ev) {
  if (from == to) return FRCNN_OK;
  FR_HIP(hipEventRecord(ev, from));
  FR_HIP(hipStreamWaitEvent(to, ev, 0));
  return FRCNN_OK;
}

static int fork_side(frcnn_model* m, hipStream_t s, size_t idx) {
  FR_TRY(ensure_side(m));
  while (m->fork_ev.size() <= idx) {
    hipEvent_t e;
    FR_HIP(hipEventCreateWithFlags(&e, hipEventDisableTiming));
    m->fork_ev.push_back(e);
  }
  FR_HIP(hipEventRecord(m->fork_ev[idx], s));
  FR_HIP(hipStreamWaitEvent(m->side, m->fork_ev[idx], 0));
  m->side_busy = true;
  return FRCNN_OK;
}

static int fork_to(frcnn_model* m, hipStream_t s, hipStream_t to, size_t idx) {
  FR_TRY(ensure_side(m));
  while (m->fork_ev.size() <= idx) {
    hipEvent_t e;
    FR_HIP(hipEventCreateWithFlags(&e, hipEventDisableTiming));
    m->fork_ev.push_back(e);
  }
  FR_HIP(hipEventRecord(m->fork_ev[idx], s));
  FR_HIP(hipStreamWaitEvent(to, m->fork_ev[idx], 0));
  m->side_busy = true;
  return FRCNN_OK;
}

static int head_forward(frcnn_model* m, Head& h, const float* w, hipStream_t s, int ws_slot) {
  const Block& in = m->blocks[h.input];
  if (h.c3.x_f)
    FR_TRY(conv_x3(in.pooled.f(), h.c3.Cin, h.c3.H, h.c3.W, nullptr, nullptr, h.c3.wx.p, w + h.c3.b_off, h.c3.Cout, h.c3.k, 0,
                   h.c3.x.f(), OUT_STORE, 0, s, ws_slot, nullptr, m->f16_packed ? m->rec(in.am) : nullptr,
                   m->f16_packed ? m->amax_ws.f() + h.c3.am : nullptr));
  else
    FR_TRY(conv_igemm(in.pooled.f(), h.c3.Cin, h.c3.H, h.c3.W, nullptr, nullptr, h.c3.wf.f(), w + h.c3.b_off,
                      h.c3.Cout, h.c3.k, 0, h.c3.x.f(), OUT_STORE, 0, s, ws_slot));
  FR_TRY(conv_igemm(h.c3.x.f(), h.c1.Cin, h.c1.H, h.c1.W, w + h.c3.a_off, nullptr, h.c1.wf.f(), w + h.c1.b_off,
                    HEAD_OUT, 1, 0, h.c1.x.f(), OUT_STORE, 0, s, ws_slot));
  return FRCNN_OK;
}

static bool any_compact(const frcnn_model* m) {
  for (auto& b : m->blocks) if (b.dc_on) return true;
  return false;
}
static bool fuse_act_on() { return !deterministic() && !(getenv("FRCNN_FUSE_ACT") && atoi(getenv("FRCNN_FUSE_ACT")) == 0); }

static int plan_compact(frcnn_model* m, int training, const float* const* drop_masks, unsigned long long seed) {
  for (auto& b : m->blocks) { b.dc_on = false; b.dc_idx = nullptr; }
  if (!training || !drop_compact_on() || !fuse_act_on() || !m->dc_pin) return FRCNN_OK;
  const unsigned slot = m->dc_step % frcnn_model::DC_RING;
  if (m->dc_ev[slot]) FR_HIP(hipEventSynchronize(m->dc_ev[slot]));
  int* idx_host = (int*)(m->dc_pin + (size_t)slot * m->dc_slot_bytes + m->dc_idx_off);
  const int* idx_dev = (const int*)((char*)m->dc_dev.p + (size_t)slot * m->dc_slot_bytes + m->dc_idx_off);
  size_t at = 0;
  std::vector<float> keep;
  for (size_t b = 0; b < m->blocks.size(); ++b) {
    Block& blk = m->blocks[b];
    const int C = m->d.filters[b];
    const size_t my = at;
    at += (size_t)C;
    if (!blk.has_drop || blk.nconv < 2) continue;
    Conv &c0 = m->convs[blk.first_conv], &c1 = m->convs[blk.first_conv + 1];
    if (!(c0.k == 3 && c1.k == 3 && c0.x_f && c1.x_f && c1.x_d && (b == 0 || c0.x_d))) continue;
    keep.resize(C);
    if (drop_masks && drop_masks[b]) {
      FR_HIP(hipMemcpy(keep.data(), drop_masks[b], (size_t)C * 4, hipMemcpyDeviceToHost));
    } else {
      for (int i = 0; i < C; ++i) keep[i] = frcnn_keep_mask(seed * 131 + b, (unsigned long long)i, blk.p_drop);
    }
    int nk = 0;
    bool binary = true;
    for (int i = 0; i < C; ++i) {
      if (keep[i] == 1.0f) idx_host[my + nk++] = i;
      else if (keep[i] != 0.0f) binary = false;
    }
    if (!binary) continue;
    for (int i = nk; i < C; ++i) idx_host[my + i] = -1;
    const int nkM = std::min(C, (nk + 63) / 64 * 64), nkK = std::min(C, (nk + 15) / 16 * 16);
    if (nk == 0 || nkK >= C) continue;
    if (!conv_x3_eligible(c0.Cin, nkM, 3) || !conv_x3_eligible(nkK, c1.Cout, 3) || !conv_x3_eligible(c1.Cout, nkM, 3) ||
        (b > 0 && !conv_x3_eligible(nkK, c0.Cin, 3)) || !conv_wgradx_eligible(nkM, c1.Cout, 3) || !conv_wgradx_eligible(c0.Cin, nkM, 3))
      continue;
    blk.dc_on = true; blk.nk = nk; blk.nkM = nkM; blk.nkK = nkK; blk.dc_idx = idx_dev + my;
  }
  return FRCNN_OK;
}

static int pack_compact(frcnn_model* m, const float* w, bool f16, hipStream_t s) {
  const unsigned slot = m->dc_step % frcnn_model::DC_RING;
  ++m->dc_step;
  char* hslot = m->dc_pin + (size_t)slot * m->dc_slot_bytes;
  char* dslot = (char*)m->dc_dev.p + (size_t)slot * m->dc_slot_bytes;
  const std::vector<PackXJob>& src = f16 ? m->x3_host16 : m->x3_host;
  PackXJob* jobs = (PackXJob*)hslot;
// ... 561 lines not shown
  FR_HIP(hipStreamWaitEvent(S(stream), m->block_rd_ev[block - 1], 0));
  return FRCNN_OK;
}

static int refresh_group(frcnn_model* m, const float* w, int group, hipStream_t s) {
  const bool f16 = get_x3_f16() && m->n_amax_jobs > 0;
  const frcnn_model::PackGroup& G = m->groups[group];
  if (G.pk_n) FR_TRY(conv_pack_weights_multi(w, (const PackJob*)m->pack_jobs.p + G.pk_off, G.pk_n, G.pk_grid, s));
  if (f16 && G.am_n) FR_TRY(tensor_absmax_multi(w, (const AmaxJob*)m->amax_jobs.p + G.am_off, G.am_n, G.am_grid, s));
  if (G.x3_n) FR_TRY(conv_x3_pack_multi(w, (const PackXJob*)m->x3_jobs.p + (f16 ? G.x3_off16 : G.x3_off), G.x3_n, G.x3_grid, s));
  return FRCNN_OK;
}
int frcnn_pnet_refresh_packs(frcnn_model* m, const float* w, int group, void* stream) {
  FR_CHECK(m->H > 0, "pnet_refresh_packs: call frcnn_pnet_forward first");
  FR_CHECK(group >= 0 && group < (int)m->groups.size(), "pnet_refresh_packs: group %d out of range", group);
  const bool f16 = get_x3_f16() && m->n_amax_jobs > 0;
  if (m->fresh_mask && (m->fresh_w != w || m->fresh_f16 != f16)) m->fresh_mask = 0;
  FR_TRY(refresh_group(m, w, group, S(stream)));
  if (group == (int)m->blocks.size()) m->head_x3_fresh = true;
  m->fresh_mask |= 1u << group; m->fresh_w = w; m->fresh_f16 = f16;
  return FRCNN_OK;
}

int frcnn_pnet_invalidate_packs(frcnn_model* m) {
  m->fresh_mask = 0;
  return FRCNN_OK;
}

int frcnn_pnet_wait_block_gradients(frcnn_model* m, int block, void* stream) {
  FR_CHECK(block >= 1 && block <= (int)m->blocks.size(), "pnet_wait_block_gradients: block %d out of range", block);
  FR_CHECK(m->block_ev_valid && (size_t)block <= m->block_ev.size(), "pnet_wait_block_gradients: call frcnn_pnet_backward first");
  FR_HIP(hipStreamWaitEvent(S(stream), m->block_ev[block - 1], 0));
  return FRCNN_OK;
}

static int record_block_read(frcnn_model* m, int b, hipStream_t s) {
  if (!m->update_armed) return FRCNN_OK;
  while (m->block_rd_ev.size() < m->blocks.size()) {
    hipEvent_t e;
    FR_HIP(hipEventCreateWithFlags(&e, hipEventDisableTiming));
    m->block_rd_ev.push_back(e);
  }
  FR_HIP(hipEventRecord(m->block_rd_ev[b], s));
  return FRCNN_OK;
}

int frcnn_pnet_backward(frcnn_model* m, const float* w, float* grad, void* stream) {
  hipStream_t s = S(stream);
  FR_CHECK(m->H > 0 && m->training, "pnet_backward: needs a preceding training-mode forward "
                                    "(nn.SpatialDropout: backprop only defined while training)");
  const int nb = (int)m->blocks.size();
  bool heads_tail = false;
  if (m->heads_begun) {
    if (!m->heads_joined) {
      static const bool partial = !(getenv("FRCNN_HEADS_PARTIAL_JOIN") && atoi(getenv("FRCNN_HEADS_PARTIAL_JOIN")) == 0);
      if (partial && m->heads_gin) {
        FR_HIP(hipStreamWaitEvent(s, m->heads_gin_ev, 0));
        heads_tail = true;
      }
      for (auto& h : m->heads) {
        if (!h.stream || m->heads_gin) continue;
        if (partial && h.gin_recorded) {
          FR_HIP(hipStreamWaitEvent(s, h.gin_done, 0));
          heads_tail = true;
        } else {
          FR_HIP(hipEventRecord(h.done, h.stream));
          FR_HIP(hipStreamWaitEvent(s, h.done, 0));
        }
      }
      if (!(partial && m->heads_gin)) {
        FR_HIP(hipEventRecord(m->join_ev, m->side));
        FR_HIP(hipStreamWaitEvent(s, m->join_ev, 0));
      }
    }
    m->heads_begun = false; m->heads_joined = false; m->side_busy = false;
  } else {
    if (m->heads_deferred) {
      bool any = false;
      for (auto& h : m->heads) any = any || h.sp_count != 0;
      if (any) FR_TRY(heads_forward_dense(m, w, s));
      m->heads_deferred = false;
    }
    FR_TRY(join_side(m, s));
    FR_TRY(fill_zero((char*)m->zero_arena.p + m->delta_bytes, m->gpool_bytes, s));
    FR_TRY(backward_heads(m, w, grad, s, 0));
  }
  {
    Block& last = m->blocks.back();
    FR_TRY(add_inplace(last.gpooled.f(), m->delta_last.f(), (long)m->d.filters[nb - 1] * last.Hp * last.Wp, s));
  }
  if (m->update_armed) {
    if (!m->bwd_ev) FR_HIP(hipEventCreateWithFlags(&m->bwd_ev, hipEventDisableTiming));
    FR_HIP(hipEventRecord(m->bwd_ev, s));
  }
  const bool use_side = side_enabled();
  if (use_side) FR_TRY(ensure_side(m));
  hipStream_t ws = use_side ? m->side : s;
  size_t n_fork = 0;
  const bool fuse_act = !deterministic() && !(getenv("FRCNN_FUSE_ACT") && atoi(getenv("FRCNN_FUSE_ACT")) == 0);
  bool act_done = false;
  for (int b = nb - 1; b >= 0; --b) {
    Block& blk = m->blocks[b];
    for (int st = blk.nconv - 1; st >= 0; --st) {
      Conv& c = m->convs[blk.first_conv + st];
      const float* scale = (st == 0 && blk.has_drop) ? blk.scale.f() : nullptr;
      const bool fused_here = act_done;
      act_done = false;
      static const bool first_pooled_on = !(getenv("FRCNN_FIRST_POOLED") && atoi(getenv("FRCNN_FIRST_POOLED")) == 0);
      const bool first_pooled = fuse_act && first_pooled_on && b == 0 && st == 0 && blk.nconv == 1 && scale == nullptr &&
                                conv_wgrad_first_pooled_eligible(c.Cin, c.Cout, c.k, c.Wo);
      if (first_pooled) {
        FR_TRY(conv_wgrad_first_pooled(m->img.f(), c.Cin, c.H, c.W, blk.gpooled.f(), (const unsigned char*)blk.pidx.p, c.x.f(),
                                       w + c.a_off, c.Cout, c.pad, grad + c.w_off, grad + c.b_off, grad + c.a_off,
                                       m->wg_ws_first.p, m->wg_ws_first.bytes, s));
        while (m->block_ev.size() < (size_t)nb) {
          hipEvent_t e;
          FR_HIP(hipEventCreateWithFlags(&e, hipEventDisableTiming));
          m->block_ev.push_back(e);
        }
        FR_HIP(hipEventRecord(m->block_ev[b], s));
        FR_TRY(record_block_read(m, b, s));
        break;
      }
      if (fused_here) {
      } else if (st == blk.nconv - 1) {
        FR_TRY(maxpool_act_backward(blk.gpooled.f(), (const unsigned char*)blk.pidx.p, c.x.f(), c.Cout, c.Ho, c.Wo,
                                    w + c.a_off, scale, c.gx.f(), grad + c.b_off, grad + c.a_off, s,
                                    (c.x_d && m->f16_packed) ? m->rec(c.am + 1) : nullptr));
      } else {
        FR_TRY(act_backward(c.gx.f(), c.x.f(), c.Cout, (long)c.Ho * c.Wo, w + c.a_off, scale, c.gx.f(),
                            grad + c.b_off, grad + c.a_off, s, (c.x_d && m->f16_packed) ? m->rec(c.am + 1) : nullptr));
      }
      const float* in; const float* in_slope = nullptr; const float* in_scale = nullptr;
      if (st > 0) {
        Conv& pc = m->convs[blk.first_conv + st - 1];
        in = pc.x.f(); in_slope = w + pc.a_off;
        in_scale = (st - 1 == 0 && blk.has_drop) ? blk.scale.f() : nullptr;
      } else {
        in = b == 0 ? m->img.f() : m->blocks[b - 1].pooled.f();
      }
      const bool dc = blk.dc_on && st <= 1;
      int wg_cin = c.Cin, wg_o = c.Cout;
      WgradMap wmap;
      if (dc) {
        wmap.Cfull = c.Cin;
        if (st == 1) { wg_cin = blk.nkM; wmap.cmap = blk.dc_idx; in_scale = nullptr; }
        else { wg_o = blk.nkM; wmap.omap = blk.dc_idx; }
      }
      const float* wa_in = nullptr; const float* wa_g = nullptr;
      if (m->f16_packed && c.x_f && c.x_d && (st > 0 || b > 0)) {
        wa_in = st > 0 ? m->rec(m->convs[blk.first_conv + st - 1].am) : m->rec(m->blocks[b - 1].am);
        wa_g = m->rec(c.am + 1);
      }
      const bool on_caller = use_side && b == 0 && st == 0;
      if (use_side && !on_caller) FR_TRY(fork_side(m, s, n_fork++));
      if (on_caller) {
        FR_TRY(conv_wgrad(in, wg_cin, c.H, c.W, in_slope, in_scale, c.gx.f(), wg_o, c.k, c.pad, grad + c.w_off, m->wg_ws_first.p,
                          m->wg_ws_first.bytes, s, fused_here ? grad + c.b_off : nullptr, wa_in, wa_g, dc ? &wmap : nullptr));
        FR_HIP(hipEventRecord(m->join_ev, ws));
        FR_HIP(hipStreamWaitEvent(s, m->join_ev, 0));
      } else {
        FR_TRY(conv_wgrad(in, wg_cin, c.H, c.W, in_slope, in_scale, c.gx.f(), wg_o, c.k, c.pad, grad + c.w_off, m->wg_ws.p, m->wg_ws.bytes, ws,
                          fused_here ? grad + c.b_off : nullptr, wa_in, wa_g, dc ? &wmap : nullptr));
      }
      if (st == 0) {
        while (m->block_ev.size() < (size_t)nb) {
          hipEvent_t e;
          FR_HIP(hipEventCreateWithFlags(&e, hipEventDisableTiming));
          m->block_ev.push_back(e);
        }
        FR_HIP(hipEventRecord(m->block_ev[b], on_caller ? s : ws));
      }
      if (b == 0 && st == 0) {
        FR_TRY(record_block_read(m, b, s));
        break;
      }
      float* gin = st > 0 ? m->convs[blk.first_conv + st - 1].gx.f() : m->blocks[b - 1].gpooled.f();
      const int gmode = st > 0 ? OUT_STORE : OUT_ADD;
      const float* ag = nullptr;
      const float* aw = nullptr;
      if (c.x_d && m->f16_packed) { ag = m->rec(c.am + 1); aw = m->amax_ws.f() + c.am; }
      const int dg_k = (dc && st == 0) ? blk.nkK : c.Cout, dg_m = (dc && st == 1) ? blk.nkM : c.Cin;
      const double fl = 2.0 * dg_k * dg_m * c.k * c.k * (double)c.Ho * c.Wo;
      if (c.x_d && st > 0 && fuse_act && c.k == 3) {
        Conv& pc = m->convs[blk.first_conv + st - 1];
        X3PostAct post{pc.x.f(), w + pc.a_off, (st - 1 == 0 && blk.has_drop && !dc) ? blk.scale.f() : nullptr, grad + pc.a_off};
        FR_TRY(conv_x3(c.gx.f(), dg_k, c.Ho, c.Wo, nullptr, nullptr, c.wxd.p, nullptr, dg_m, c.k, c.k - 1 - c.pad, gin, gmode, fl, s, 0, &post, ag, aw,
                       (pc.x_d && m->f16_packed) ? m->rec(pc.am + 1) : nullptr));
        act_done = true;
      } else if (c.x_d)
        FR_TRY(conv_x3(c.gx.f(), dg_k, c.Ho, c.Wo, nullptr, nullptr, c.wxd.p, nullptr, dg_m, c.k, c.k - 1 - c.pad, gin, gmode, fl, s, 0, nullptr, ag, aw));
      else
        FR_TRY(conv_igemm(c.gx.f(), c.Cout, c.Ho, c.Wo, nullptr, nullptr, c.wd.f(), nullptr, c.Cin, c.k,
                          c.k - 1 - c.pad, gin, gmode, fl, s));
      if (st == 0) FR_TRY(record_block_read(m, b, s));
    }
  }
  m->block_ev_valid = true;
  if (heads_tail && !m->heads_gin) FR_TRY(join_heads(m, s));
  FR_TRY(cw_join(m, s));
  if (use_side) {
    FR_HIP(hipEventRecord(m->join_ev, ws));
    FR_HIP(hipStreamWaitEvent(s, m->join_ev, 0));
    m->side_busy = false;
  }
  return FRCNN_OK;
}

static bool cnet_fuse() {
  const char* e = getenv("FRCNN_CNET_FUSE");
  return !(e && atoi(e) == 0);
}
static bool gemm_f16_on() {
  static const bool env_on = !(getenv("FRCNN_GEMM_F16") && atoi(getenv("FRCNN_GEMM_F16")) == 0);
  return env_on && get_x3_f16();
}
static int ensure_cnet(frcnn_model* m, int R) {
  for (auto& L : m->cls) {
    size_t n = (size_t)R * L.n * 4;
    FR_TRY(L.lin.ensure(n));
    if (L.bn) { FR_TRY(L.pre.ensure(n)); FR_TRY(L.xhat.ensure(n)); FR_TRY(L.invstd.ensure((size_t)L.n * 4)); }
    FR_TRY(L.post.ensure(n));
    FR_TRY(L.g.ensure(n));
    FR_TRY(L.gin.ensure((size_t)R * L.in * 4));
    if (L.p_drop > 0.f) FR_TRY(L.mask.ensure(n));
    L.x_form = 0;
    for (int role : {1, 2, 4}) if (linear_x_eligible(role, R, L.in, L.n)) L.x_form |= role;
    const size_t Rp = (size_t)linear_x_rows_padded(R);
    if (L.x_form & 1) FR_TRY(L.xp.ensure((size_t)3 * R * L.in * 2));
    if (L.x_form & 2) FR_TRY(L.gp.ensure((size_t)3 * R * L.n * 2));
    if (L.x_form & 4) { FR_TRY(L.xpT.ensure((size_t)3 * L.in * Rp * 2)); FR_TRY(L.gpT.ensure((size_t)3 * L.n * Rp * 2)); }
    if (L.x_form & 7) FR_TRY(L.am.ensure((size_t)5 * AMAX_REC * 4));
  }
  int nc = m->d.class_count + 1;
  int nf = m->cls.empty() ? m->D : m->cls.back().n;
  FR_TRY(m->feat_g.ensure((size_t)R * nf * 4));
  FR_TRY(m->logits.ensure((size_t)R * nc * 4));
  FR_TRY(m->lsm.ensure((size_t)R * nc * 4));
  FR_TRY(m->glog.ensure((size_t)R * nc * 4));
  return FRCNN_OK;
}

int frcnn_cnet_forward(frcnn_model* m, const float* weights, const float* x, int R, int training,
                       const float* const* drop_masks, unsigned long long seed, float* bn_running,
                       float* bbox_out, float* cls_out, void* stream) {
  hipStream_t s = S(stream);
  FR_CHECK(R > 0, "cnet_forward: empty batch");
  FR_TRY(cw_join(m, s));
  FR_TRY(ensure_cnet(m, R));
  m->R = R; m->cnet_x = x; m->training = training;
  const float* w = weights;
  const float* cur = x;
  float* bnr = bn_running;
  for (size_t l = 0; l < m->cls.size(); ++l) {
    ClsLayer& L = m->cls[l];
    GemmFold fold;
    GemmFold* defer = cnet_fuse() ? &fold : nullptr;
    if ((L.x_form & 3) && gemm_f16_on()) {
      float* rw = L.am.f() + 2 * AMAX_REC;
      const bool have = !training && g_static_weights && L.am_w_gen == g_static_gen && L.am_w_of == w;
      if (!have) FR_TRY(tensor_absmax(w + L.w_off, (long)L.n * L.in, rw, s));
      L.am_w_of = w; L.am_w_gen = training ? -1 : g_static_gen;
    } else {
      L.am_w_of = nullptr;
    }
    if ((L.x_form & 1) && gemm_f16_on()) {
      float* rx = L.am.f();
      FR_TRY(tensor_absmax(cur, (long)R * L.in, rx, s));
      FR_TRY(split_planes(cur, R, L.in, L.xp.p, nullptr, s, rx));
      FR_TRY(linear_x_forward(L.xp.p, R, L.in, w + L.w_off, w + L.b_off, L.n, L.lin.f(), s, 0, defer, rx, rx + 2 * AMAX_REC));
    } else if (L.x_form & 1) {
      FR_TRY(split_planes(cur, R, L.in, L.xp.p, nullptr, s));
      FR_TRY(linear_x_forward(L.xp.p, R, L.in, w + L.w_off, w + L.b_off, L.n, L.lin.f(), s, 0, defer));
    } else {
      FR_TRY(gemm_f32(cur, L.in, 1, w + L.w_off, 1, L.in, L.lin.f(), L.n, R, L.n, L.in, OUT_STORE, w + L.b_off, s, 0, defer));
    }
    if (L.bn) FR_CHECK(training || bnr, "cnet_forward: evaluate mode needs bn_running");
    const float* mask = nullptr;
    float inv_keep = 1.f;
    bool draw = false;
    if (training && L.p_drop > 0.f) {
      inv_keep = 1.0f / (1.0f - L.p_drop);
      if (drop_masks && drop_masks[l])
        FR_HIP(hipMemcpyAsync(L.mask.p, drop_masks[l], (size_t)R * L.n * 4, hipMemcpyDeviceToDevice, s));
      else
        draw = true;
      mask = L.mask.f();
    }
    if (defer) {
      FR_TRY(cnet_act_forward(L.lin.f(), fold, R, L.n, L.bn ? w + L.bnw_off : nullptr, L.bn ? w + L.bnb_off : nullptr, L.bn ? bnr : nullptr,
                              training, L.lin.f(), L.xhat.f(), L.invstd.f(), L.pre.f(), w + L.a_off, const_cast<float*>(mask), draw,
                              inv_keep, L.p_drop, seed * 977 + l + 17, L.post.f(), s));
      if (L.bn && bnr) bnr += 2 * L.n;
      cur = L.post.f();
      continue;
    }
    const float* pre = L.lin.f();
    if (L.bn) {
      FR_TRY(bn_forward(L.lin.f(), R, L.n, w + L.bnw_off, w + L.bnb_off, bnr, training, L.xhat.f(), L.invstd.f(),
                        L.pre.f(), s));
      if (bnr) bnr += 2 * L.n;
      pre = L.pre.f();
    }
    if (draw)
      FR_TRY(prelu_dropout_forward_gen(pre, (long)R * L.n, w + L.a_off, L.mask.f(), L.p_drop, seed * 977 + l + 17,
                                       L.post.f(), s));
    else
      FR_TRY(prelu_dropout_forward(pre, (long)R * L.n, w + L.a_off, mask, inv_keep, L.post.f(), s));
    cur = L.post.f();
  }
  const int nf = m->cls.empty() ? m->D : m->cls.back().n;
  const int nc = m->d.class_count + 1;
  if (cnet_fuse() && cnet_heads_fused_eligible(nf, nc)) {
    return cnet_heads_forward(cur, R, nf, w + m->bbox_w_off, w + m->bbox_b_off, w + m->clsw_off, w + m->clsb_off, nc, bbox_out,
                              m->logits.f(), m->lsm.f(), cls_out, s);
  }
// ... 132 lines not shown
```

faster-rcnn.torch_amd/csrc/wgradx.hip:

```cpp
#include <cstdlib>

#include "kernels.h"
#include "amax.h"
#include <type_traits>

namespace frcnn {

typedef float f32x16 __attribute__((ext_vector_type(16)));
typedef __bf16 bf16x8 __attribute__((ext_vector_type(8)));
typedef __bf16 bf16x4 __attribute__((ext_vector_type(4)));
typedef __bf16 bf16x2 __attribute__((ext_vector_type(2)));
typedef float f32x2 __attribute__((ext_vector_type(2)));
typedef _Float16 f16x8 __attribute__((ext_vector_type(8)));
typedef _Float16 f16x2 __attribute__((ext_vector_type(2)));

#define WX_TH 4
#define WX_TW 16
#define WX_GROW 128
#define WX_GPLANE (64 * WX_GROW)
#define WX_XROW 48
#define WX_XCH (6 * WX_XROW)
#define WX_XPLANE (64 * WX_XCH + 8 * 16)
#define WX_LDS (3 * WX_GPLANE + 3 * WX_XPLANE)

bool conv_wgradx_eligible(int Cin, int O, int k) {
  return get_split_bf16() && k == 3 && Cin % 64 == 0 && O % 64 == 0;
}

__device__ __forceinline__ unsigned wx_cvt2(float a, float b) {
  f32x2 v = {a, b};
  bf16x2 r = __builtin_convertvector(v, bf16x2);
  return __builtin_bit_cast(unsigned, r);
}
__device__ __forceinline__ void wx_split4(const float* v, uint2& H, uint2& Mi, uint2& L) {
  unsigned h[2], m[2], l[2];
#pragma unroll
  for (int j = 0; j < 2; ++j) {
    const float x0 = v[2 * j], x1 = v[2 * j + 1];
    h[j] = wx_cvt2(x0, x1);
    const float r0 = x0 - __builtin_bit_cast(float, h[j] << 16), r1 = x1 - __builtin_bit_cast(float, h[j] & 0xFFFF0000u);
    m[j] = wx_cvt2(r0, r1);
    const float s0 = r0 - __builtin_bit_cast(float, m[j] << 16), s1 = r1 - __builtin_bit_cast(float, m[j] & 0xFFFF0000u);
    l[j] = wx_cvt2(s0, s1);
  }
  H = make_uint2(h[0], h[1]); Mi = make_uint2(m[0], m[1]); L = make_uint2(l[0], l[1]);
}

__device__ __forceinline__ unsigned wx_cvt2h(float a, float b) {
  f32x2 v = {a, b};
  f16x2 r = __builtin_convertvector(v, f16x2);
  return __builtin_bit_cast(unsigned, r);
}
__device__ __forceinline__ int wx_exp(float amax, int top) {
  const int be = (int)((__builtin_bit_cast(unsigned, amax) >> 23) & 0xFFu);
  if (be == 0 || be == 255) return 0;
  const int e = top - (be - 127);
  return e < -100 ? -100 : e > 100 ? 100 : e;
}
__device__ __forceinline__ float wx_pow2(int e) { return __builtin_bit_cast(float, (unsigned)(e + 127) << 23); }

struct WgradXArgs {
  const float* in;
  const float* in_slope;
  const float* in_scale;
  const float* g;
  float* slab;
  float* gbias;
  const float* amax_in;
  const float* amax_g;
  const int* omap;
  int Cin, H, W, O, Ho, Wo, pad;
  int tilesX, tilesY, oTiles, cTiles, nSplit;
};

__device__ __forceinline__ unsigned wx_xaddr(int c) { return (unsigned)(c * WX_XCH + (c >> 3) * 16); }
__device__ __forceinline__ unsigned wx_gswz(int o) { const unsigned u = (o >> 1) & 7; return ((u & 3) << 1) | (u >> 2); }

typedef unsigned u32x4 __attribute__((ext_vector_type(4)));
typedef float f32x4u __attribute__((ext_vector_type(4), aligned(4)));

#define WX_PIN(x) asm volatile("" : "+v"(x))

template <int N, class F>
__device__ __forceinline__ void static_for(F&& f) {
  if constexpr (N > 0) {
    static_for<N - 1>(f);
    f(std::integral_constant<int, N - 1>{});
  }
}

template <bool SLOPE, bool SCALE, int VEC, int NP = 3>
__global__ __launch_bounds__(256, 1) void conv_wgradx_kernel(WgradXArgs p) {
  extern __shared__ __attribute__((aligned(16))) char smem[];
  constexpr unsigned LDSI = NP * (WX_GPLANE + WX_XPLANE), XB = NP * WX_GPLANE;
  const int tid = threadIdx.x, lane = tid & 63;
  const int wave = __builtin_amdgcn_readfirstlane(tid >> 6);
  const int wo = wave >> 1, wc = wave & 1;
  const int h = lane >> 5, li = lane & 31;

  int bid;
  {
    const int nblk = gridDim.x, xcd = blockIdx.x & 7, idx = blockIdx.x >> 3;
    const int q = nblk >> 3, r = nblk & 7;
    bid = xcd * q + min(xcd, r) + idx;
  }
  const int ot = bid % p.oTiles; bid /= p.oTiles;
  const int ct = bid % p.cTiles;
  const int split = bid / p.cTiles;
  const int o0 = ot * 64, c0 = ct * 64;
  const int HW = p.H * p.W, HoWo = p.Ho * p.Wo;
  const float slope = SLOPE ? *p.in_slope : 1.f;
  float gmul = 1.f, xmul = 1.f, out_mul = 1.f, out_mul2 = 1.f;
  if (NP == 2) {
    const float ag = amax_load_block(p.amax_g);
    float ax = amax_load_block(p.amax_in);
    if (SLOPE) ax *= fmaxf(1.f, fabsf(slope));
    const int eg = wx_exp(ag, 14), ex = wx_exp(ax, SCALE ? 13 : 14);
    gmul = wx_pow2(eg); xmul = wx_pow2(ex);
    const int et = -(eg + ex), e1 = et / 2;
    out_mul = wx_pow2(e1); out_mul2 = wx_pow2(et - e1);
  }

  f32x16 acc[9];
#pragma unroll
  for (int t = 0; t < 9; ++t)
#pragma unroll
    for (int r = 0; r < 16; ++r) acc[t][r] = 0.f;

  const int srow = tid >> 2, sq = tid & 3;
  const float* const gsrc = p.g + (size_t)(o0 + srow) * HoWo;
  const float* const xsrc = p.in + (size_t)(c0 + srow) * HW;
  auto gat = [&](int elem_off) { return gsrc + elem_off; };
  auto xat = [&](int elem_off) { return xsrc + elem_off; };
  const float xscale = SCALE ? p.in_scale[c0 + srow] : 1.f;
  const unsigned gdst = (unsigned)(srow * WX_GROW) + ((((unsigned)sq >> 1) ^ wx_gswz(srow)) << 4) + (sq & 1) * 8;
  const unsigned xdst = XB + wx_xaddr(srow) + sq * 8;
  int xr[9], xs[9];
#pragma unroll
  for (int k = 0; k < 9; ++k) {
    const int j = sq + 4 * k;
    xr[k] = j / 6; xs[k] = j - 6 * xr[k];
  }

  const int oA = wo * 32 + li, cB = wc * 32 + li;
  const unsigned abase = (unsigned)(oA * WX_GROW) + (((unsigned)h ^ wx_gswz(oA)) << 4);
  const unsigned bbase = XB + wx_xaddr(cB) + h * 16;

  const int nPix = p.tilesX * p.tilesY;
  const int nT = (nPix - split + p.nSplit - 1) / p.nSplit;
  struct Pre {
    float vg[4][4], vx[9][4];
    bool ok[13];
    int oy0, ox0;
  };
#ifdef WX_ONE_SET
  Pre pre[1];
#else
  Pre pre[2];
#endif
  float sr[13][4];
  unsigned sh[13][2], sm[13][2], sl[13][2];
  float bsum = 0.f;
  bool bsum_on = true;
  auto up_lo = [](unsigned v) { return __builtin_bit_cast(float, v << 16); };
  auto up_hi = [](unsigned v) { return __builtin_bit_cast(float, v & 0xFFFF0000u); };
  const int adv_y = p.nSplit / p.tilesX, adv_x = p.nSplit % p.tilesX;
  int w_ty = split / p.tilesX, w_tx = split % p.tilesX, w_i = 0;
  auto load_origin = [&](Pre& P) {
    P.oy0 = w_ty * WX_TH; P.ox0 = w_tx * WX_TW;
    const int more = w_i + 1 < nT ? 1 : 0;
    w_tx += more * adv_x; w_ty += more * adv_y;
    const int wrap = w_tx >= p.tilesX ? 1 : 0;
    w_tx -= wrap * p.tilesX; w_ty += wrap;
    ++w_i;
  };
  auto load_step = [&](auto itc, Pre& P) {
    constexpr int it = decltype(itc)::value;
    const int oy0 = P.oy0, ox0 = P.ox0;
    if constexpr (it < 4) {
      constexpr int k = it;
      const int oy = oy0 + k, ox = ox0 + 4 * sq;
      if (VEC) {
        P.ok[it] = oy < p.Ho && ox < p.Wo;
        const f32x4u v = *reinterpret_cast<const f32x4u*>(gat((oy * p.Wo + ox) & -(int)P.ok[it]));
        P.vg[k][0] = v[0]; P.vg[k][1] = v[1]; P.vg[k][2] = v[2]; P.vg[k][3] = v[3];
      } else {
#pragma unroll
        for (int e = 0; e < 4; ++e) P.vg[k][e] = *gat((oy * p.Wo + ox + e) & -(int)(oy < p.Ho && ox + e < p.Wo));
      }
    } else {
      constexpr int k = it - 4;
      const int iy = oy0 - p.pad + xr[k], ix = ox0 - p.pad - 3 + 4 * xs[k];
      if (VEC) {
        P.ok[it] = (unsigned)iy < (unsigned)p.H && (unsigned)ix < (unsigned)p.W;
        const f32x4u v = *reinterpret_cast<const f32x4u*>(xat((iy * p.W + ix) & -(int)P.ok[it]));
        P.vx[k][0] = v[0]; P.vx[k][1] = v[1]; P.vx[k][2] = v[2]; P.vx[k][3] = v[3];
      } else {
#pragma unroll
        for (int e = 0; e < 4; ++e)
          P.vx[k][e] = *xat((iy * p.W + ix + e) & -(int)((unsigned)iy < (unsigned)p.H && (unsigned)(ix + e) < (unsigned)p.W));
      }
    }
  };
  auto inside = [&](auto itc, int e, Pre& P) -> bool {
    constexpr int it = decltype(itc)::value;
    if (VEC == 1) return P.ok[it];
    if (VEC == 2) {
      if constexpr (it < 4) return P.ok[it] && P.ox0 + 4 * sq + e < p.Wo;
      else return P.ok[it] && P.ox0 - p.pad - 3 + 4 * xs[it < 4 ? 0 : it - 4] + e < p.W;
    }
    if constexpr (it < 4) return P.oy0 + it < p.Ho && P.ox0 + 4 * sq + e < p.Wo;
    else return (unsigned)(P.oy0 - p.pad + xr[it < 4 ? 0 : it - 4]) < (unsigned)p.H &&
                (unsigned)(P.ox0 - p.pad - 3 + 4 * xs[it < 4 ? 0 : it - 4] + e) < (unsigned)p.W;
  };
  constexpr int XPH0 = (SLOPE || SCALE) ? 0 : 4;
  auto stage_step = [&](auto itc, auto phc, unsigned gwb, unsigned xwb, Pre& P) {
    constexpr int it = decltype(itc)::value, ph = decltype(phc)::value;
    if constexpr (ph < 4) {
      constexpr int k = it - 4;
      {
        constexpr int e = ph;
        float v = P.vx[k][e];
        if (SLOPE) v = v > 0.f ? v : slope * v;
        if (SCALE) v *= xscale;
        P.vx[k][e] = inside(itc, e, P) ? v : 0.f;
        WX_PIN(P.vx[k][e]);
      }
    } else if constexpr (ph == 4 || ph == 6) {
      constexpr int j = (ph - 4) / 2;
      float x0 = it < 4 ? P.vg[it < 4 ? it : 0][2 * j] : P.vx[it < 4 ? 0 : it - 4][2 * j];
      float x1 = it < 4 ? P.vg[it < 4 ? it : 0][2 * j + 1] : P.vx[it < 4 ? 0 : it - 4][2 * j + 1];
      if (it < 4 || XPH0 == 4) {
        x0 = inside(itc, 2 * j, P) ? x0 : 0.f;
        x1 = inside(itc, 2 * j + 1, P) ? x1 : 0.f;
      }
      if (it < 4) bsum += bsum_on ? x0 + x1 : 0.f;
      if constexpr (NP == 2) {
        const float mul = it < 4 ? gmul : xmul;
        x0 *= mul; x1 *= mul;
        sh[it][j] = wx_cvt2h(x0, x1);
        const f16x2 hv = __builtin_bit_cast(f16x2, sh[it][j]);
        sr[it][2 * j] = x0 - (float)hv[0];
        sr[it][2 * j + 1] = x1 - (float)hv[1];
      } else {
        sh[it][j] = wx_cvt2(x0, x1);
        sr[it][2 * j] = x0 - up_lo(sh[it][j]);
        sr[it][2 * j + 1] = x1 - up_hi(sh[it][j]);
      }
      WX_PIN(sh[it][j]); WX_PIN(sr[it][2 * j]); WX_PIN(sr[it][2 * j + 1]);
    } else if constexpr (ph == 5 || ph == 7) {
      constexpr int j = (ph - 5) / 2;
      if constexpr (NP == 2) {
        sl[it][j] = wx_cvt2h(sr[it][2 * j], sr[it][2 * j + 1]);
        WX_PIN(sl[it][j]);
      } else {
        sm[it][j] = wx_cvt2(sr[it][2 * j], sr[it][2 * j + 1]);
        const float s0 = sr[it][2 * j] - up_lo(sm[it][j]), s1 = sr[it][2 * j + 1] - up_hi(sm[it][j]);
        sl[it][j] = wx_cvt2(s0, s1);
        WX_PIN(sm[it][j]); WX_PIN(sl[it][j]);
      }
    } else {
      char* d = it < 4 ? smem + (gwb ^ ((unsigned)it << 5)) : smem + xwb + 32 * (it - 4);
      constexpr int PL = it < 4 ? WX_GPLANE : WX_XPLANE;
      *reinterpret_cast<uint2*>(d) = make_uint2(sh[it][0], sh[it][1]);
      if constexpr (NP == 2) {
        *reinterpret_cast<uint2*>(d + PL) = make_uint2(sl[it][0], sl[it][1]);
      } else {
        *reinterpret_cast<uint2*>(d + PL) = make_uint2(sm[it][0], sm[it][1]);
        *reinterpret_cast<uint2*>(d + 2 * PL) = make_uint2(sl[it][0], sl[it][1]);
      }
      asm volatile("" ::: "memory");
    }
  };
  auto stage_seq = [&](auto i0c, auto sc, unsigned gwb, unsigned xwb, Pre& P) {
    constexpr int I0 = decltype(i0c)::value, s = decltype(sc)::value;
    constexpr int NG = I0 < 4 ? 4 - I0 : 0;
    constexpr int NPX = 9 - XPH0;
    constexpr int it = s < 5 * NG ? I0 + s / 5 : I0 + NG + (s - 5 * NG) / NPX;
    constexpr int ph = s < 5 * NG ? 4 + s % 5 : XPH0 + (s - 5 * NG) % NPX;
    stage_step(std::integral_constant<int, it>{}, std::integral_constant<int, ph>{}, gwb, xwb, P);
  };

  u32x4 a[WX_TH][NP];
  u32x4 b[3][NP], bn[3][NP];
  u32x4 raw[NP][2];
  constexpr int NQ = NP == 2 ? 3 : 6;
  constexpr int PA[6] = {NP == 2 ? 1 : 2, 0, NP == 2 ? 0 : 1, 1, 0, 0}, PB[6] = {0, NP == 2 ? 1 : 2, NP == 2 ? 0 : 1, 0, 1, 0};
  auto read_row = [&](unsigned rb, int r) {
    if (r < WX_TH) {
#pragma unroll
      for (int pl = 0; pl < NP; ++pl)
        a[r][pl] = *reinterpret_cast<const u32x4*>(smem + rb + pl * WX_GPLANE + (abase ^ ((unsigned)r << 5)));
    }
#pragma unroll
    for (int pl = 0; pl < NP; ++pl) {
      raw[pl][0] = *reinterpret_cast<const u32x4*>(smem + rb + bbase + pl * WX_XPLANE + r * WX_XROW);
      raw[pl][1] = *reinterpret_cast<const u32x4*>(smem + rb + bbase + pl * WX_XPLANE + r * WX_XROW + 16);
    }
  };
  auto cut_step = [&](auto sc) {
    constexpr int pl = decltype(sc)::value >> 1, hf = decltype(sc)::value & 1;
    const u32x4 d0 = raw[pl][0], d1 = raw[pl][1];
    const unsigned d[8] = {d0[0], d0[1], d0[2], d0[3], d1[0], d1[1], d1[2], d1[3]};
    if (hf == 1) asm volatile("" ::"v"(d[0]), "v"(d[7]));
#pragma unroll
    for (int j = 2 * hf; j < 2 * hf + 2; ++j) {
      bn[0][pl][j] = __builtin_amdgcn_alignbit(d[j + 2], d[j + 1], 16);
      bn[1][pl][j] = d[j + 2];
      bn[2][pl][j] = __builtin_amdgcn_alignbit(d[j + 3], d[j + 2], 16);
      WX_PIN(bn[0][pl][j]); WX_PIN(bn[1][pl][j]); WX_PIN(bn[2][pl][j]);
    }
  };

  load_origin(pre[0]);
  static_for<13>([&](auto itc) { load_step(itc, pre[0]); });
  constexpr int NST = 4 * 5 + 9 * (9 - XPH0);
  static_for<NST>([&](auto sc) { stage_seq(std::integral_constant<int, 0>{}, sc, gdst, xdst, pre[0]); });
  __syncthreads();
#ifdef WX_ONE_SET
  load_origin(pre[0]);
  static_for<13>([&](auto itc) { load_step(itc, pre[0]); });
#else
  load_origin(pre[1]);
  static_for<13>([&](auto itc) { load_step(itc, pre[1]); });
  load_origin(pre[0]);
  static_for<13>([&](auto itc) { load_step(itc, pre[0]); });
#endif
  read_row(0, 0);
  static_for<2 * NP>([&](auto sc) { cut_step(sc); });
#pragma unroll
  for (int kx = 0; kx < 3; ++kx)
#pragma unroll
    for (int pl = 0; pl < NP; ++pl) b[kx][pl] = bn[kx][pl];

  auto tile = [&](int i, Pre& P) {
    const unsigned rb = (i & 1) ? LDSI : 0, wb = LDSI - rb;
    const unsigned gwb = gdst + wb, xwb = xdst + wb;
    bsum_on = i + 1 < nT;
    auto row = [&](auto rc) {
      constexpr int r = decltype(rc)::value;
      constexpr int nky = r < 3 ? r + 1 : 6 - r;
      constexpr int NM = 3 * NQ * nky;
      constexpr int NPX = 9 - XPH0;
      constexpr int NSTG = r == 1 ? 4 * 5 + NPX : (r == 2 || r == 3) ? 4 * NPX : r == 4 ? 13 : 0;
      constexpr int NS = NSTG + 2 * NP;
      __builtin_amdgcn_sched_barrier(0);
      if (r < 5) read_row(rb, r + 1); else read_row(wb, 0);
      __builtin_amdgcn_sched_barrier(0);
      static_for<NM>([&](auto mc) {
        constexpr int m = decltype(mc)::value;
        constexpr int q = m / (3 * nky), kyi = (m / 3) % nky, kx = m % 3;
        constexpr int ky = (r < WX_TH ? 0 : r - (WX_TH - 1)) + kyi, ks = r - ky;
        static_assert(ks >= 0 && ks < WX_TH && ky < 3, "tap walk");
        if constexpr (NP == 2)
          acc[3 * ky + kx] = __builtin_amdgcn_mfma_f32_32x32x16_f16(__builtin_bit_cast(f16x8, a[ks][PA[q]]), __builtin_bit_cast(f16x8, b[kx][PB[q]]), acc[3 * ky + kx], 0, 0, 0);
        else
          acc[3 * ky + kx] = __builtin_amdgcn_mfma_f32_32x32x16_bf16(__builtin_bit_cast(bf16x8, a[ks][PA[q]]), __builtin_bit_cast(bf16x8, b[kx][PB[q]]), acc[3 * ky + kx], 0, 0, 0);
        __builtin_amdgcn_sched_barrier(0);
        constexpr int LEAD = NSTG == 0 ? 6 : 0;
        constexpr int s0 = m < LEAD ? 0 : (m - LEAD) * NS / (NM - LEAD), s1 = m < LEAD ? 0 : (m - LEAD + 1) * NS / (NM - LEAD);
        static_for<s1 - s0>([&](auto dc) {
          constexpr int s = s0 + decltype(dc)::value;
          if constexpr (s >= NSTG) {
            cut_step(std::integral_constant<int, s - NSTG>{});
          } else if constexpr (r >= 1 && r <= 3) {
            stage_seq(std::integral_constant<int, r == 1 ? 0 : r == 2 ? 5 : 9>{}, std::integral_constant<int, s>{}, gwb, xwb, P);
          } else {
            if constexpr (s == 0) load_origin(P);
            load_step(std::integral_constant<int, s>{}, P);
          }
        });
        __builtin_amdgcn_sched_barrier(0);
      });
#pragma unroll
      for (int kx = 0; kx < 3; ++kx)
#pragma unroll
        for (int pl = 0; pl < NP; ++pl) b[kx][pl] = bn[kx][pl];
      if (r == 4) __syncthreads();
    };
    row(std::integral_constant<int, 0>{}); row(std::integral_constant<int, 1>{}); row(std::integral_constant<int, 2>{});
    row(std::integral_constant<int, 3>{}); row(std::integral_constant<int, 4>{}); row(std::integral_constant<int, 5>{});
  };
  {
    int i = 0;
#ifdef WX_ONE_SET
    for (; i < nT; ++i) tile(i, pre[0]);
#else
    for (; i + 1 < nT; i += 2) { tile(i, pre[1]); tile(i + 1, pre[0]); }
    if (i < nT) tile(i, pre[1]);
#endif
  }
  if (p.gbias && ct == 0) {
    float v = bsum;
    v += __shfl_xor(v, 1); v += __shfl_xor(v, 2);
    const int od = p.omap ? p.omap[o0 + srow] : o0 + srow;
    if (sq == 0 && od >= 0) unsafeAtomicAdd(p.gbias + od, v);
  }
  {
    const int c = c0 + wc * 32 + li;
    const size_t OC = (size_t)p.O * p.Cin;
    float* sl = p.slab + (size_t)split * 9 * OC;
#pragma unroll
    for (int tap = 0; tap < 9; ++tap)
#pragma unroll
      for (int r = 0; r < 16; ++r) {
        const int o = o0 + wo * 32 + (r & 3) + 8 * (r >> 2) + 4 * h;
        sl[(size_t)tap * OC + (size_t)o * p.Cin + c] = NP == 2 ? (acc[tap][r] * out_mul) * out_mul2 : acc[tap][r];
      }
  }
}

static void wgradx_plan(WgradXArgs& a) {
  a.tilesX = cdiv(a.Wo, WX_TW); a.tilesY = cdiv(a.Ho, WX_TH);
  a.oTiles = a.O / 64; a.cTiles = a.Cin / 64;
  const long base = (long)a.oTiles * a.cTiles, npix = (long)a.tilesX * a.tilesY;
  a.nSplit = (int)std::max<long>(1, std::min<long>(npix, 256 / base));
  if (const char* e = getenv("FRCNN_WGX_NSPLIT")) a.nSplit = (int)std::max<long>(1, std::min<long>(npix, atoi(e)));
}

size_t conv_wgradx_workspace_bytes(int Cin, int H, int W, int O, int pad) {
  WgradXArgs a;
  a.Cin = Cin; a.H = H; a.W = W; a.O = O; a.pad = pad; a.Ho = H + 2 * pad - 2; a.Wo = W + 2 * pad - 2;
  wgradx_plan(a);
  return (size_t)a.nSplit * 9 * O * Cin * 4 + 256;
}

static const WgradMap* g_wx_map = nullptr;

template <bool SLOPE, bool SCALE, int VEC, int NP = 3>
static int launch_wgradx_v(WgradXArgs& a, double flops, float* gw, hipStream_t s) {
  static bool attr_set = false;
  if (!attr_set) {
    FR_HIP(hipFuncSetAttribute(reinterpret_cast<const void*>(conv_wgradx_kernel<SLOPE, SCALE, VEC, NP>),
                               hipFuncAttributeMaxDynamicSharedMemorySize, NP == 2 ? 120 * 1024 : 160 * 1024));
    attr_set = true;
  }
  const int grid = a.oTiles * a.cTiles * a.nSplit;
  const double bytes = 4.0 * ((double)a.Cin * a.H * a.W + (double)a.O * a.Ho * a.Wo);
  if (prof_enabled(KC_CONV_WGRADX)) prof_before(KC_CONV_WGRADX, s);
  const size_t lds = 2 * (size_t)NP * (WX_GPLANE + WX_XPLANE);
  hipLaunchKernelGGL((conv_wgradx_kernel<SLOPE, SCALE, VEC, NP>), dim3(grid), dim3(256), lds, s, a);
  if (g_wx_map) FR_TRY(wgrad_reduce_map(a.slab, a.nSplit, 9, a.O, a.Cin, gw, *g_wx_map, s));
  else FR_TRY(wgrad_reduce(a.slab, a.nSplit, 9, a.O * a.Cin, gw, s));
  if (prof_enabled(KC_CONV_WGRADX)) prof_after(KC_CONV_WGRADX, flops, bytes, s);
  FR_LAUNCH_CHECK();
  return FRCNN_OK;
}

static bool readable_past_end(const void* p, size_t bytes, size_t slack) {
  hipDeviceptr_t base = nullptr;
  size_t size = 0;
  if (hipMemGetAddressRange(&base, &size, (hipDeviceptr_t)p) != hipSuccess) { (void)hipGetLastError(); return false; }
  return (uintptr_t)p + bytes + slack <= (uintptr_t)base + size;
}

template <bool SLOPE, bool SCALE, int NP = 3>
static int launch_wgradx(WgradXArgs& a, double flops, float* gw, hipStream_t s) {
  if (a.pad == 1 && a.W % 4 == 0 && ((uintptr_t)a.in & 15) == 0 && ((uintptr_t)a.g & 15) == 0)
    return launch_wgradx_v<SLOPE, SCALE, 1, NP>(a, flops, gw, s);
  if (a.pad == 1 && readable_past_end(a.in, (size_t)a.Cin * a.H * a.W * 4, 12) && readable_past_end(a.g, (size_t)a.O * a.Ho * a.Wo * 4, 12))
    return launch_wgradx_v<SLOPE, SCALE, 2, NP>(a, flops, gw, s);
  return launch_wgradx_v<SLOPE, SCALE, 0, NP>(a, flops, gw, s);
}

int conv_wgradx(const float* in, int Cin, int H, int W, const float* in_slope, const float* in_scale, const float* g, int O,
                int pad, float* gw, void* ws, size_t ws_bytes, hipStream_t s, float* gbias, const float* amax_in, const float* amax_g,
                const WgradMap* map) {
  WgradXArgs a;
  a.in = in; a.in_slope = in_slope; a.in_scale = in_scale; a.g = g; a.gbias = gbias;
  a.amax_in = amax_in; a.amax_g = amax_g;
  a.omap = map ? map->omap : nullptr;
  struct MapScope { MapScope(const WgradMap* m) { g_wx_map = (m && (m->omap || m->cmap)) ? m : nullptr; } ~MapScope() { g_wx_map = nullptr; } } scope(map);
  FR_CHECK((amax_in != nullptr) == (amax_g != nullptr), "conv_wgradx: the fp16 form needs the magnitude records of both tensors");
  a.Cin = Cin; a.H = H; a.W = W; a.O = O; a.pad = pad; a.Ho = H + 2 * pad - 2; a.Wo = W + 2 * pad - 2;
  FR_CHECK(Cin % 64 == 0 && O % 64 == 0, "conv_wgradx: %d channels x %d filters is not a split-bf16 shape", Cin, O);
  FR_CHECK((long)Cin * H * W < (1L << 30) && (long)O * a.Ho * a.Wo < (1L << 30), "conv_wgradx: tensor too large for 32-bit offsets");
  wgradx_plan(a);
  const size_t need = (size_t)a.nSplit * 9 * O * Cin * 4 + 256;
  FR_CHECK(ws && ws_bytes >= need, "conv_wgradx: workspace too small (%zu < %zu)", ws_bytes, need);
  a.slab = (float*)(((uintptr_t)ws + 255) / 256 * 256);
  const double flops = 2.0 * O * Cin * 9 * (double)a.Ho * a.Wo;
  if (amax_in) {
    if (in_slope) return in_scale ? launch_wgradx<true, true, 2>(a, flops, gw, s) : launch_wgradx<true, false, 2>(a, flops, gw, s);
    return in_scale ? launch_wgradx<false, true, 2>(a, flops, gw, s) : launch_wgradx<false, false, 2>(a, flops, gw, s);
  }
  if (in_slope) return in_scale ? launch_wgradx<true, true>(a, flops, gw, s) : launch_wgradx<true, false>(a, flops, gw, s);
  return in_scale ? launch_wgradx<false, true>(a, flops, gw, s) : launch_wgradx<false, false>(a, flops, gw, s);
}

}
```

include/frcnn_hip.h:

```cpp
#ifndef FRCNN_HIP_H
#define FRCNN_HIP_H

#include <stddef.h>

#ifdef __cplusplus
extern "C" {
#endif

#define FRCNN_OK 0
#define FRCNN_ERR_ARG 1
#define FRCNN_ERR_HIP 2
#define FRCNN_ERR_STATE 3

int frcnn_version(void);
const char *frcnn_last_error(void);
int frcnn_device_count(int *n);
int frcnn_set_device(int device);
int frcnn_device_name(char *buf_host, int len);
int frcnn_set_option(const char *name, int value);
int frcnn_get_option(const char *name, int *value_host);

int frcnn_malloc(void **ptr_out_host, size_t bytes);
int frcnn_free(void *ptr);
int frcnn_host_alloc(void **ptr_out_host, size_t bytes);
int frcnn_host_free(void *ptr_host);
int frcnn_memcpy_h2d(void *dst, const void *src_host, size_t bytes, void *stream);
int frcnn_memcpy_d2h(void *dst_host, const void *src, size_t bytes, void *stream);
int frcnn_memcpy_d2d(void *dst, const void *src, size_t bytes, void *stream);
int frcnn_stream_sync(void *stream);
int frcnn_zero(void *ptr, size_t bytes, void *stream);
int frcnn_scale(float *x, long long n, float s, void *stream);
int frcnn_add(float *y, const float *x, long long n, void *stream);

#define FRCNN_KC_CONV_IGEMM_K3 0
#define FRCNN_KC_CONV_IGEMM_OTHER 1
#define FRCNN_KC_CONV_WGRAD_K3 2
#define FRCNN_KC_CONV_WGRAD_OTHER 3
#define FRCNN_KC_GEMM 4
#define FRCNN_KC_ELEMWISE 5
#define FRCNN_KC_ROI 6
#define FRCNN_KC_RPN 7
#define FRCNN_KC_NMS 8
#define FRCNN_KC_OPTIM 9
#define FRCNN_KC_IMAGE 10
#define FRCNN_KC_CONV_X3 11
#define FRCNN_KC_CONV_WGRADX 12
#define FRCNN_KC_COUNT 13
int frcnn_prof_enable(int class_mask);
int frcnn_prof_collect(long long *launches_host, double *ms_host, double *flops_host,
                       double *bytes_host);

size_t frcnn_nms_workspace_bytes(int n);
int frcnn_nms_device(const float *boxes, int n, int ncols, float overlap, int key_mode,
                     int key_col, long long *pick, int *count, void *workspace,
                     size_t workspace_bytes, void *stream);
int frcnn_nms_device_classes(const float *boxes, int n, int ncols, float overlap, int key_mode, int key_col,
                             const int *cls, long long *pick, int *count, void *workspace,
                             size_t workspace_bytes, void *stream);
int frcnn_nms_device_n(const float *boxes, int n_cap, const int *n_dev, int ncols, float overlap, int key_mode, int key_col,
                       const int *cls, long long *pick, int *count, void *workspace, size_t workspace_bytes, void *stream);
int frcnn_roi_windows(const double *rect, const long long *pick, int k, const int *layers_host, int nlayers, int fmH, int fmW,
                      int *wins, void *stream);
int frcnn_detect_post(const int *cls, const float *conf, const float *bbox, const double *rect, const long long *pick, int R,
                      int bgclass, double min_conf, float *bb, int *kc, int *keep_row, double *r2, int *K_dev, void *stream);
int frcnn_detect_gather(const long long *wpick, const int *nwin_dev, int cap, const int *keep_row, const int *kc,
                        const float *bb, const double *r2, const long long *pick, const float *match_p,
                        const double *match_rect, const int *match_idx, double *rec, void *stream);
int frcnn_nms_host(const float *boxes_host, int n, int ncols, float overlap, int key_mode,
                   int key_col, long long *pick_host, int *count_host);

int frcnn_conv2d_forward(const float *in, int C, int H, int W, const float *in_slope,
                         const float *in_scale, const float *weight, const float *bias, int O,
                         int k, int pad, float *out, void *stream);
int frcnn_conv2d_backward_input(const float *gout, int O, int Ho, int Wo, const float *weight,
                                int C, int k, int pad, float *gin, int accumulate, void *stream);
int frcnn_conv2d_backward_weight(const float *in, int C, int H, int W, const float *in_slope,
                                 const float *in_scale, const float *gout, int O, int k, int pad,
                                 float *gweight, float *gbias, void *stream);

int frcnn_maxpool_act_forward(const float *x, int C, int H, int W, const float *slope,
                              const float *scale, float *out, unsigned char *idx, void *stream);
int frcnn_maxpool_act_backward(const float *gpool, const unsigned char *idx, const float *x, int C,
                               int H, int W, const float *slope, const float *scale, float *gx,
                               float *gbias, float *gslope, void *stream);
int frcnn_act_forward(const float *x, int C, long long hw, const float *slope, const float *scale,
                      float *y, void *stream);
int frcnn_act_backward(const float *gy, const float *x, int C, long long hw, const float *slope,
                       const float *scale, float *gx, float *gbias, float *gslope, void *stream);

int frcnn_roi_pool_forward(const float *fmap, int C, int H, int W, const int *wins, int R, int kh,
                           int kw, float *out, int *idx, void *stream);
int frcnn_roi_pool_backward(float *gmap, int C, int H, int W, const float *gout, const int *idx,
                            int R, int kh, int kw, void *stream);

size_t frcnn_rpn_scan_workspace_bytes(const int *H_host, const int *W_host);
int frcnn_rpn_scan(const float *const *maps_host, const int *H_host, const int *W_host,
                   const float *anchor_w, const float *anchor_h, double img_w, double img_h,
                   double p_threshold, int cap, float *match_p, int *match_idx,
                   double *match_rect, float *match_box, int *count, void *workspace,
                   size_t workspace_bytes, void *stream);

int frcnn_rpn_loss(const float *const *maps_host, float *const *deltas_host, const int *H_host,
                   const int *W_host, const int *ex_idx, const double *ex_anchor,
                   const double *ex_roi, const int *ex_class, int npos, int nneg, int bgclass,
                   double *ex_loss, float *crtarget, float *cctarget, void *stream);

int frcnn_loss_accumulate(const double *ex_loss, int E, double *acc, void *stream);

int frcnn_linear_forward(const float *x, int R, int I, const float *weight, const float *bias,
                         int O, float *y, void *stream);
int frcnn_linear_backward(const float *x, const float *gy, int R, int I, const float *weight,
                          int O, float *gx, float *gweight, float *gbias, void *stream);

int frcnn_rmsprop(float *x, const float *g, float *m, long long n, float lr, float alpha,
                  float eps, void *stream);
int frcnn_scale_rmsprop(float *x, float *g, float gscale, float *m, long long n, float lr, float alpha,
                        float eps, void *stream);
int frcnn_scale_rmsprop_dev(float *x, float *g, const double *gcount_dev, float *m, long long n, float lr,
                            float alpha, float eps, void *stream);
int frcnn_scale_rmsprop_slice(float *x, float *g, float gscale, float *m, long long lo, long long hi, float lr,
                              float alpha, float eps, void *stream);

typedef struct {
  int nblocks;
  int filters[8], ksize[8], pad[8], conv_steps[8];
  float dropout[8];
  int nheads;
  int head_k[8], head_n[8], head_input[8];
  int ncls;
  int cls_n[8], cls_bn[8];
  float cls_dropout[8];
  int class_count;
  int kh, kw;
} frcnn_model_desc;

typedef struct frcnn_model frcnn_model;

int frcnn_model_create(const frcnn_model_desc *desc_host, frcnn_model **out_host);
int frcnn_model_destroy(frcnn_model *);
int frcnn_model_param_count(const frcnn_model *, long long *total_host, long long *pnet_host);
int frcnn_model_param_table(const frcnn_model *, long long *table_host, int cap, int *n_host);
int frcnn_model_localizer_layers(const frcnn_model *, int output_index, int *layers_host, int cap,
                                 int *n_host);

int frcnn_pnet_forward(frcnn_model *, const float *weights, const float *img, int H, int W,
                       int training, const float *const *drop_masks_host, unsigned long long seed,
                       void *stream);
int frcnn_pnet_forward_async_heads(frcnn_model *, const float *weights, const float *img, int H, int W,
                                   const float *const *drop_masks_host, unsigned long long seed,
                                   void *stream);
int frcnn_pnet_output(frcnn_model *, int i, float **ptr_host, int *C_host, int *H_host,
                      int *W_host);
int frcnn_model_debug_buffer(frcnn_model *, int kind, int index, void **ptr_host, long long *bytes_host);
int frcnn_pnet_delta(frcnn_model *, int i, float **ptr_host);
int frcnn_pnet_zero_deltas(frcnn_model *, void *stream);
int frcnn_pnet_set_sparse_deltas(frcnn_model *, int head, const int *positions, int count);
int frcnn_pnet_backward_heads_begin(frcnn_model *, const float *weights, float *grad, void *stream);
int frcnn_pnet_anchor_loss_begin(frcnn_model *, const float *weights, float *grad, const int *ex_idx,
                                 const double *ex_anchor, const double *ex_roi, const int *ex_class,
                                 int npos, int nneg, int bgclass, double *ex_loss, float *crtarget,
                                 float *cctarget, double *acc, void *stream);
int frcnn_pnet_anchor_loss_wait(frcnn_model *, void *stream);
int frcnn_pnet_backward_heads_join(frcnn_model *, void *stream, int *joined_host);
int frcnn_pnet_backward(frcnn_model *, const float *weights, float *grad, void *stream);

int frcnn_pnet_wait_block_gradients(frcnn_model *, int block, void *stream);

int frcnn_model_update_stream(frcnn_model *, void **stream_host);
int frcnn_model_update_fork(frcnn_model *, void *stream);
int frcnn_model_update_join(frcnn_model *, void *stream);
int frcnn_pnet_wait_backward_begun(frcnn_model *, void *stream);
int frcnn_pnet_wait_heads_done(frcnn_model *, void *stream);
int frcnn_pnet_wait_block_done(frcnn_model *, int block, void *stream);
int frcnn_pnet_refresh_packs(frcnn_model *, const float *weights, int group, void *stream);
int frcnn_pnet_invalidate_packs(frcnn_model *);

int frcnn_cnet_forward(frcnn_model *, const float *weights, const float *x, int R, int training,
                       const float *const *drop_masks_host, unsigned long long seed,
                       float *bn_running, float *bbox_out, float *cls_out, void *stream);
int frcnn_cnet_backward_join(frcnn_model *, void *stream);
int frcnn_cnet_backward(frcnn_model *, const float *weights, const float *g_bbox,
                        const float *g_cls, float *gx, float *grad, void *stream);
int frcnn_cnet_losses(float *crout, const float *crtarget, const float *ccout,
                      const float *cctarget, int R, int npos, int ncls, float *crdelta,
                      float *ccdelta, double *loss2, void *stream);
int frcnn_cnet_decode(const float *cls_out, int R, int ncls, int *cls, float *conf, void *stream);

int frcnn_image_rgb2yuv(const float *rgb, float *yuv, int H, int W, void *stream);
int frcnn_image_rgb2hsv(const float *rgb, float *hsv, int H, int W, void *stream);
int frcnn_image_rgb2lab(const float *rgb, float *lab, int H, int W, void *stream);
int frcnn_image_scale(const float *src, int C, int H, int W, float *dst, int dH, int dW, float *tmp,
                      int rgb2yuv, void *stream);
int frcnn_image_scale_u8(const unsigned char *src_hwc, int H, int W, float *dst, int dH, int dW,
                         float *tmp, int rgb2yuv, void *stream);
int frcnn_image_crop_flip(const float *src, int C, int H, int W, int x0, int y0, int w, int h, int hflip,
                          int vflip, float *dst, void *stream);
size_t frcnn_image_normalize_workspace_bytes(int C);
int frcnn_image_normalize(float *img, int C, int H, int W, int centering, int scaling, void *workspace,
                          size_t workspace_bytes, void *stream);
int frcnn_image_contrastive_norm(const float *in, int H, int W, const float *kernel_host, int K,
                                 float threshold, float *out, float *tmp, void *stream);

typedef struct frcnn_anchors frcnn_anchors;
int frcnn_anchors_create(const float *w_tab_host, const float *h_tab_host, const double *cx_host,
                         const double *cy_host, int nscales, int width, frcnn_anchors **out_host);
int frcnn_anchors_destroy(frcnn_anchors *);
int frcnn_anchors_assemble(frcnn_anchors *, const double *rois_host, int nroi, double img_w, double img_h,
                           double pos_thr, double neg_thr, int best_match, int nearby_aversion,
                           int negatives, unsigned int *mt_state_host, int *mt_index_host, int *ex_host,
                           double *ex_rect_host, int cap, int *npos_host, int *nneg_host);

#define FRCNN_COMM_ID_BYTES 128
typedef struct frcnn_comm frcnn_comm;
int frcnn_comm_get_unique_id(void *id_host);
int frcnn_comm_exchange_id_file(const char *path, int rank, void *id_host, int timeout_ms);
int frcnn_comm_init_rank(frcnn_comm **out_host, int nranks, int rank, const void *id_host);
int frcnn_comm_init_rank_timeout(frcnn_comm **out_host, int nranks, int rank, const void *id_host, int timeout_ms);
int frcnn_comm_init_rank_file(frcnn_comm **out_host, int nranks, int rank, const char *path, int timeout_ms);
int frcnn_comm_destroy(frcnn_comm *);
int frcnn_comm_info(const frcnn_comm *, int *nranks_host, int *rank_host);
int frcnn_comm_query(const frcnn_comm *, int *count_host, int *user_rank_host, int *device_host);
int frcnn_allreduce_f32(frcnn_comm *, float *buf, long long n, void *stream);
int frcnn_allreduce_f64(frcnn_comm *, double *buf, long long n, void *stream);
int frcnn_broadcast_f32(frcnn_comm *, float *buf, long long n, int root, void *stream);

#ifdef __cplusplus
}
#endif
#endif
```

Baseline: 534.5.

## Use 2:4 sparse MFMA for weight gradient of convs feeding a maxpool

```diff
diff --git a/faster-rcnn.torch_amd/_lib.py b/faster-rcnn.torch_amd/_lib.py
--- a/faster-rcnn.torch_amd/_lib.py
+++ b/faster-rcnn.torch_amd/_lib.py
@@ -60,6 +60,7 @@
     "frcnn_conv2d_forward": ([vp, C.c_int, C.c_int, C.c_int, vp, vp, vp, vp, C.c_int, C.c_int, C.c_int, vp, vp], C.c_int),
     "frcnn_conv2d_backward_input": ([vp, C.c_int, C.c_int, C.c_int, vp, C.c_int, C.c_int, C.c_int, vp, C.c_int, vp], C.c_int),
     "frcnn_conv2d_backward_weight": ([vp, C.c_int, C.c_int, C.c_int, vp, vp, vp, C.c_int, C.c_int, C.c_int, vp, vp, vp], C.c_int),
+    "frcnn_conv2d_backward_weight_pooled": ([vp, C.c_int, C.c_int, C.c_int, vp, vp, vp, C.c_int, C.c_int, C.c_int, vp, vp, vp], C.c_int),
     "frcnn_maxpool_act_forward": ([vp, C.c_int, C.c_int, C.c_int, vp, vp, vp, vp, vp], C.c_int),
     "frcnn_maxpool_act_backward": ([vp, vp, vp, C.c_int, C.c_int, C.c_int, vp, vp, vp, vp, vp, vp], C.c_int),
     "frcnn_act_forward": ([vp, C.c_int, C.c_longlong, vp, vp, vp, vp], C.c_int),
diff --git a/faster-rcnn.torch_amd/csrc/api.cpp b/faster-rcnn.torch_amd/csrc/api.cpp
--- a/faster-rcnn.torch_amd/csrc/api.cpp
+++ b/faster-rcnn.torch_amd/csrc/api.cpp
@@ -268,9 +268,9 @@
   (void)hipFree(wd);
   return rc;
 }
-int frcnn_conv2d_backward_weight(const float* in, int C, int H, int W, const float* in_slope,
-                                 const float* in_scale, const float* gout, int O, int k, int pad,
-                                 float* gweight, float* gbias, void* stream) {
+static int conv2d_backward_weight(const float* in, int C, int H, int W, const float* in_slope,
+                                  const float* in_scale, const float* gout, int O, int k, int pad,
+                                  float* gweight, float* gbias, void* stream, bool pooled) {
   size_t wsb = conv_wgrad_workspace_bytes(C, H, W, O, k, pad);
   void* ws = nullptr;
   FR_HIP(hipMalloc(&ws, wsb));
@@ -284,7 +284,8 @@
     if (rc == FRCNN_OK) rc = tensor_absmax(gout, (long)O * (H + 2 * pad - k + 1) * (W + 2 * pad - k + 1), am + AMAX_REC, S(stream));
   }
   if (rc == FRCNN_OK)
-    rc = conv_wgrad(in, C, H, W, in_slope, in_scale, gout, O, k, pad, gweight, ws, wsb, S(stream), nullptr, am, am ? am + AMAX_REC : nullptr);
+    rc = conv_wgrad(in, C, H, W, in_slope, in_scale, gout, O, k, pad, gweight, ws, wsb, S(stream), nullptr, am, am ? am + AMAX_REC : nullptr,
+                    nullptr, pooled);
   (void)hipStreamSynchronize(S(stream));
   (void)hipFree(ws); (void)hipFree(am);
   FR_TRY(rc);
@@ -293,6 +294,16 @@
     FR_TRY(channel_sum(gout, O, (long)Ho * Wo, gbias, S(stream)));
   }
   return FRCNN_OK;
+}
+int frcnn_conv2d_backward_weight(const float* in, int C, int H, int W, const float* in_slope,
+                                 const float* in_scale, const float* gout, int O, int k, int pad,
+                                 float* gweight, float* gbias, void* stream) {
+  return conv2d_backward_weight(in, C, H, W, in_slope, in_scale, gout, O, k, pad, gweight, gbias, stream, false);
+}
+int frcnn_conv2d_backward_weight_pooled(const float* in, int C, int H, int W, const float* in_slope,
+                                        const float* in_scale, const float* gout, int O, int k, int pad,
+                                        float* gweight, float* gbias, void* stream) {
+  return conv2d_backward_weight(in, C, H, W, in_slope, in_scale, gout, O, k, pad, gweight, gbias, stream, true);
 }
 
 int frcnn_maxpool_act_forward(const float* x, int C, int H, int W, const float* slope, const float* scale,
diff --git a/faster-rcnn.torch_amd/csrc/conv.hip b/faster-rcnn.torch_amd/csrc/conv.hip
--- a/faster-rcnn.torch_amd/csrc/conv.hip
+++ b/faster-rcnn.torch_amd/csrc/conv.hip
@@ -1271,13 +1271,13 @@
 
 int conv_wgrad(const float* in, int Cin, int H, int W, const float* in_slope, const float* in_scale,
                const float* g, int O, int k, int pad, float* gw, void* ws, size_t ws_bytes, hipStream_t s, float* gbias,
-               const float* amax_in, const float* amax_g, const WgradMap* map) {
+               const float* amax_in, const float* amax_g, const WgradMap* map, bool pooled) {
   WgradArgs a;
   a.in = in; a.in_slope = in_slope; a.in_scale = in_scale; a.g = g;
   a.Cin = Cin; a.H = H; a.W = W; a.O = O; a.pad = pad;
   a.Ho = H + 2 * pad - k + 1; a.Wo = W + 2 * pad - k + 1;
   FR_CHECK(k == 1 || k == 3 || k == 5 || k == 7, "conv_wgrad: unsupported kernel size %d", k);
-  if (conv_wgradx_eligible(Cin, O, k)) return conv_wgradx(in, Cin, H, W, in_slope, in_scale, g, O, pad, gw, ws, ws_bytes, s, gbias, amax_in, amax_g, map);
+  if (conv_wgradx_eligible(Cin, O, k)) return conv_wgradx(in, Cin, H, W, in_slope, in_scale, g, O, pad, gw, ws, ws_bytes, s, gbias, amax_in, amax_g, map, pooled);
   FR_CHECK(!map || (!map->omap && !map->cmap), "conv_wgrad: a gathered weight gradient needs a conv_wgradx shape");
   if (gbias) FR_TRY(channel_sum(g, O, (long)a.Ho * a.Wo, gbias, s));
   FR_CHECK((long)Cin * H * W < (1L << 31) && (long)O * a.Ho * a.Wo < (1L << 31), "conv_wgrad: tensor too large for 32-bit offsets");
diff --git a/faster-rcnn.torch_amd/csrc/kernels.h b/faster-rcnn.torch_amd/csrc/kernels.h
--- a/faster-rcnn.torch_amd/csrc/kernels.h
+++ b/faster-rcnn.torch_amd/csrc/kernels.h
@@ -60,7 +60,7 @@
 int conv_wgradx(const float* in, int Cin, int H, int W, const float* in_slope, const float* in_scale, const float* g, int O,
                 int pad, float* gw, void* ws, size_t ws_bytes, hipStream_t s, float* gbias = nullptr,
                 const float* amax_in = nullptr, const float* amax_g = nullptr,
-                const WgradMap* map = nullptr);
+                const WgradMap* map = nullptr, bool pooled = false);
 int wgrad_reduce(const float* slab, int nSplit, int taps, int OC, float* gw, hipStream_t s);
 int wgrad_reduce_map(const float* slab, int nSplit, int taps, int O, int C, float* gw, const WgradMap& map, hipStream_t s);
 bool conv_wgrad_first_pooled_eligible(int Cin, int O, int k, int Wo);
@@ -73,7 +73,9 @@
                const float* g, int O, int k, int pad, float* gw, void* ws, size_t ws_bytes, hipStream_t s,
                float* gbias = nullptr,
                const float* amax_in = nullptr, const float* amax_g = nullptr,
-               const WgradMap* map = nullptr);
+               const WgradMap* map = nullptr,
+               bool pooled = false);
+bool sparse_wgrad_on();
 
 bool deterministic();
 void set_deterministic(bool on);
diff --git a/faster-rcnn.torch_amd/csrc/net.cpp b/faster-rcnn.torch_amd/csrc/net.cpp
--- a/faster-rcnn.torch_amd/csrc/net.cpp
+++ b/faster-rcnn.torch_amd/csrc/net.cpp
@@ -92,6 +92,11 @@
 static int drop_compact_on() {
   if (g_drop_compact < 0) g_drop_compact = getenv("FRCNN_DROP_COMPACT") ? (atoi(getenv("FRCNN_DROP_COMPACT")) != 0) : 1;
   return g_drop_compact;
+}
+static int g_sparse_wgrad = -1;
+bool frcnn::sparse_wgrad_on() {
+  if (g_sparse_wgrad < 0) g_sparse_wgrad = getenv("FRCNN_SPARSE_WGRAD") ? (atoi(getenv("FRCNN_SPARSE_WGRAD")) != 0) : 1;
+  return g_sparse_wgrad;
 }
 static int pool_stream(int slot, hipStream_t* out) {
   static hipStream_t pool[8] = {};
@@ -672,6 +677,7 @@
   if (strcmp(name, "deterministic") == 0) { *value = deterministic() ? 1 : 0; return FRCNN_OK; }
   if (strcmp(name, "static_weights") == 0) { *value = g_static_weights; return FRCNN_OK; }
   if (strcmp(name, "drop_compact") == 0) { *value = drop_compact_on(); return FRCNN_OK; }
+  if (strcmp(name, "sparse_wgrad") == 0) { *value = sparse_wgrad_on(); return FRCNN_OK; }
   if (strcmp(name, "sparse_heads") == 0) { *value = sparse_heads_on(); return FRCNN_OK; }
   if (strcmp(name, "winograd") == 0) { *value = 0; return FRCNN_OK; }
   if (strcmp(name, "cnet_wgrad_async") == 0) { *value = g_cnet_wgrad_async; return FRCNN_OK; }
@@ -687,6 +693,7 @@
   if (strcmp(name, "deterministic") == 0) { set_deterministic(value != 0); return FRCNN_OK; }
   if (strcmp(name, "static_weights") == 0) { g_static_weights = value != 0; ++g_static_gen; return FRCNN_OK; }
   if (strcmp(name, "drop_compact") == 0) { g_drop_compact = value != 0; return FRCNN_OK; }
+  if (strcmp(name, "sparse_wgrad") == 0) { g_sparse_wgrad = value != 0; return FRCNN_OK; }
   if (strcmp(name, "sparse_heads") == 0) { g_sparse_heads = value != 0; return FRCNN_OK; }
   if (strcmp(name, "gemm_x_roles") == 0) { set_gemm_x_roles(value); return FRCNN_OK; }
   if (strcmp(name, "split_bf16") == 0) { set_split_bf16(value); return FRCNN_OK; }
@@ -1554,16 +1561,17 @@
         wa_in = st > 0 ? m->rec(m->convs[blk.first_conv + st - 1].am) : m->rec(m->blocks[b - 1].am);
         wa_g = m->rec(c.am + 1);
       }
+      const bool pooled = !fused_here && st == blk.nconv - 1;
       const bool on_caller = use_side && b == 0 && st == 0;
       if (use_side && !on_caller) FR_TRY(fork_side(m, s, n_fork++));
       if (on_caller) {
         FR_TRY(conv_wgrad(in, wg_cin, c.H, c.W, in_slope, in_scale, c.gx.f(), wg_o, c.k, c.pad, grad + c.w_off, m->wg_ws_first.p,
-                          m->wg_ws_first.bytes, s, fused_here ? grad + c.b_off : nullptr, wa_in, wa_g, dc ? &wmap : nullptr));
+                          m->wg_ws_first.bytes, s, fused_here ? grad + c.b_off : nullptr, wa_in, wa_g, dc ? &wmap : nullptr, pooled));
         FR_HIP(hipEventRecord(m->join_ev, ws));
         FR_HIP(hipStreamWaitEvent(s, m->join_ev, 0));
       } else {
         FR_TRY(conv_wgrad(in, wg_cin, c.H, c.W, in_slope, in_scale, c.gx.f(), wg_o, c.k, c.pad, grad + c.w_off, m->wg_ws.p, m->wg_ws.bytes, ws,
-                          fused_here ? grad + c.b_off : nullptr, wa_in, wa_g, dc ? &wmap : nullptr));
+                          fused_here ? grad + c.b_off : nullptr, wa_in, wa_g, dc ? &wmap : nullptr, pooled));
       }
       if (st == 0) {
         while (m->block_ev.size() < (size_t)nb) {
diff --git a/faster-rcnn.torch_amd/csrc/wgradx.hip b/faster-rcnn.torch_amd/csrc/wgradx.hip
--- a/faster-rcnn.torch_amd/csrc/wgradx.hip
+++ b/faster-rcnn.torch_amd/csrc/wgradx.hip
@@ -22,6 +22,9 @@
 #define WX_XCH (6 * WX_XROW)
 #define WX_XPLANE (64 * WX_XCH + 8 * 16)
 #define WX_LDS (3 * WX_GPLANE + 3 * WX_XPLANE)
+#define WX_GROW_S 64
+#define WX_GPLANE_S (64 * WX_GROW_S)
+#define WX_IPLANE (64 * 8)
 
 bool conv_wgradx_eligible(int Cin, int O, int k) {
   return get_split_bf16() && k == 3 && Cin % 64 == 0 && O % 64 == 0;
@@ -75,8 +78,12 @@
 
 __device__ __forceinline__ unsigned wx_xaddr(int c) { return (unsigned)(c * WX_XCH + (c >> 3) * 16); }
 __device__ __forceinline__ unsigned wx_gswz(int o) { const unsigned u = (o >> 1) & 7; return ((u & 3) << 1) | (u >> 2); }
+__device__ __forceinline__ unsigned wx_gswz_s(int o) { return (unsigned)(o >> 2) & 3; }
 
 typedef unsigned u32x4 __attribute__((ext_vector_type(4)));
+typedef unsigned u32x8 __attribute__((ext_vector_type(8)));
+typedef _Float16 f16x16 __attribute__((ext_vector_type(16)));
+typedef __bf16 bf16x16 __attribute__((ext_vector_type(16)));
 typedef float f32x4u __attribute__((ext_vector_type(4), aligned(4)));
 
 #define WX_PIN(x) asm volatile("" : "+v"(x))
@@ -89,10 +96,12 @@
   }
 }
 
-template <bool SLOPE, bool SCALE, int VEC, int NP = 3>
+template <bool SLOPE, bool SCALE, int VEC, int NP = 3, bool GSP = false>
 __global__ __launch_bounds__(256, 1) void conv_wgradx_kernel(WgradXArgs p) {
   extern __shared__ __attribute__((aligned(16))) char smem[];
-  constexpr unsigned LDSI = NP * (WX_GPLANE + WX_XPLANE), XB = NP * WX_GPLANE;
+  constexpr unsigned GPL = GSP ? WX_GPLANE_S : WX_GPLANE, IB = NP * GPL;
+  constexpr unsigned XB = IB + (GSP ? WX_IPLANE : 0), LDSI = XB + NP * WX_XPLANE;
+  static_assert(LDSI % 128 == 0, "the row XOR of the staging addresses survives the image offset");
   const int tid = threadIdx.x, lane = tid & 63;
   const int wave = __builtin_amdgcn_readfirstlane(tid >> 6);
   const int wo = wave >> 1, wc = wave & 1;
@@ -133,7 +142,9 @@
   auto gat = [&](int elem_off) { return gsrc + elem_off; };
   auto xat = [&](int elem_off) { return xsrc + elem_off; };
   const float xscale = SCALE ? p.in_scale[c0 + srow] : 1.f;
-  const unsigned gdst = (unsigned)(srow * WX_GROW) + ((((unsigned)sq >> 1) ^ wx_gswz(srow)) << 4) + (sq & 1) * 8;
+  const unsigned gdst = GSP ? (unsigned)(srow * WX_GROW_S) + (wx_gswz_s(srow) << 4) + sq * 4
+                            : (unsigned)(srow * WX_GROW) + ((((unsigned)sq >> 1) ^ wx_gswz(srow)) << 4) + (sq & 1) * 8;
+  const unsigned idst = IB + srow * 8 + 4 * (sq & 1) + 2 * (sq >> 1);
   const unsigned xdst = XB + wx_xaddr(srow) + sq * 8;
   int xr[9], xs[9];
 #pragma unroll
@@ -143,7 +154,9 @@
   }
 
   const int oA = wo * 32 + li, cB = wc * 32 + li;
-  const unsigned abase = (unsigned)(oA * WX_GROW) + (((unsigned)h ^ wx_gswz(oA)) << 4);
+  const unsigned abase = GSP ? (unsigned)(oA * WX_GROW_S) + (((unsigned)h ^ wx_gswz_s(oA)) << 4)
+                             : (unsigned)(oA * WX_GROW) + (((unsigned)h ^ wx_gswz(oA)) << 4);
+  const unsigned ibase = IB + oA * 8 + 4 * h;
   const unsigned bbase = XB + wx_xaddr(cB) + h * 16;
 
   const int nPix = p.tilesX * p.tilesY;
@@ -160,6 +173,7 @@
 #endif
   float sr[13][4];
   unsigned sh[13][2], sm[13][2], sl[13][2];
+  unsigned iw[2];
   float bsum = 0.f;
   bool bsum_on = true;
   auto up_lo = [](unsigned v) { return __builtin_bit_cast(float, v << 16); };
@@ -216,7 +230,67 @@
   constexpr int XPH0 = (SLOPE || SCALE) ? 0 : 4;
   auto stage_step = [&](auto itc, auto phc, unsigned gwb, unsigned xwb, Pre& P) {
     constexpr int it = decltype(itc)::value, ph = decltype(phc)::value;
-    if constexpr (ph < 4) {
+    if constexpr (GSP && it < 4) {
+      constexpr int k = it < 4 ? it : 0;
+      if constexpr (ph == 4) {
+        float v[4];
+#pragma unroll
+        for (int e = 0; e < 4; ++e) v[e] = inside(itc, e, P) ? P.vg[k][e] : 0.f;
+        bsum += bsum_on ? v[0] + v[1] : 0.f;
+        bsum += bsum_on ? v[2] + v[3] : 0.f;
+        const bool n1 = v[1] != 0.f, n3 = v[3] != 0.f;
+        sr[it][0] = n1 ? v[1] : v[0];
+        sr[it][1] = n3 ? v[3] : v[2];
+        const unsigned nib = (8u | (n1 ? 1u : 0u) | (n3 ? 4u : 0u)) << (16 * (k >> 1) + 4 * sq);
+        iw[k & 1] = k < 2 ? nib : iw[k & 1] | nib;
+        WX_PIN(sr[it][0]); WX_PIN(sr[it][1]); WX_PIN(iw[k & 1]);
+      } else if constexpr (ph == 5) {
+        float x0 = sr[it][0], x1 = sr[it][1];
+        if constexpr (NP == 2) {
+          x0 *= gmul; x1 *= gmul;
+          sh[it][0] = wx_cvt2h(x0, x1);
+          const f16x2 hv = __builtin_bit_cast(f16x2, sh[it][0]);
+          sr[it][0] = x0 - (float)hv[0]; sr[it][1] = x1 - (float)hv[1];
+        } else {
+          sh[it][0] = wx_cvt2(x0, x1);
+          sr[it][0] = x0 - up_lo(sh[it][0]); sr[it][1] = x1 - up_hi(sh[it][0]);
+        }
+        WX_PIN(sh[it][0]); WX_PIN(sr[it][0]); WX_PIN(sr[it][1]);
+      } else if constexpr (ph == 6) {
+        if constexpr (NP == 2) {
+          sl[it][0] = wx_cvt2h(sr[it][0], sr[it][1]);
+          WX_PIN(sl[it][0]);
+        } else {
+          sm[it][0] = wx_cvt2(sr[it][0], sr[it][1]);
+          sr[it][0] -= up_lo(sm[it][0]); sr[it][1] -= up_hi(sm[it][0]);
+          WX_PIN(sm[it][0]); WX_PIN(sr[it][0]); WX_PIN(sr[it][1]);
+        }
+      } else if constexpr (ph == 7) {
+        if constexpr (NP == 3) {
+          sl[it][0] = wx_cvt2(sr[it][0], sr[it][1]);
+          WX_PIN(sl[it][0]);
+        }
+      } else {
+        char* d = smem + (gwb ^ ((unsigned)k << 4));
+        *reinterpret_cast<unsigned*>(d) = sh[it][0];
+        if constexpr (NP == 2) {
+          *reinterpret_cast<unsigned*>(d + GPL) = sl[it][0];
+        } else {
+          *reinterpret_cast<unsigned*>(d + GPL) = sm[it][0];
+          *reinterpret_cast<unsigned*>(d + 2 * GPL) = sl[it][0];
+        }
+        if constexpr (k == 3) {
+          unsigned w0 = iw[0], w1 = iw[1];
+          w0 |= (unsigned)__builtin_amdgcn_update_dpp(0, (int)w0, 0xB1, 0xF, 0xF, false);
+          w1 |= (unsigned)__builtin_amdgcn_update_dpp(0, (int)w1, 0xB1, 0xF, 0xF, false);
+          w0 |= (unsigned)__builtin_amdgcn_update_dpp(0, (int)w0, 0x4E, 0xF, 0xF, false);
+          w1 |= (unsigned)__builtin_amdgcn_update_dpp(0, (int)w1, 0x4E, 0xF, 0xF, false);
+          const unsigned w = (sq & 1) ? w1 : w0;
+          *reinterpret_cast<unsigned short*>(smem + (gwb - gdst) + idst) = (unsigned short)(w >> (16 * (sq >> 1)));
+        }
+        asm volatile("" ::: "memory");
+      }
+    } else if constexpr (ph < 4) {
       constexpr int k = it - 4;
       {
         constexpr int e = ph;
@@ -281,9 +355,12 @@
     stage_step(std::integral_constant<int, it>{}, std::integral_constant<int, ph>{}, gwb, xwb, P);
   };
 
-  u32x4 a[WX_TH][NP];
+  u32x4 a[GSP ? 2 : WX_TH][NP];
   u32x4 b[3][NP], bn[3][NP];
   u32x4 raw[NP][2];
+  u32x8 bt[3][NP], btn[3][NP];
+  u32x4 raw1[NP][2];
+  unsigned idxv[2] = {0, 0};
   constexpr int NQ = NP == 2 ? 3 : 6;
   constexpr int PA[6] = {NP == 2 ? 1 : 2, 0, NP == 2 ? 0 : 1, 1, 0, 0}, PB[6] = {0, NP == 2 ? 1 : 2, NP == 2 ? 0 : 1, 0, 1, 0};
   auto read_row = [&](unsigned rb, int r) {
@@ -310,6 +387,53 @@
       bn[2][pl][j] = __builtin_amdgcn_alignbit(d[j + 3], d[j + 2], 16);
       WX_PIN(bn[0][pl][j]); WX_PIN(bn[1][pl][j]); WX_PIN(bn[2][pl][j]);
     }
+  };
+
+  auto read_prow = [&](u32x4 (&dst)[NP][2], unsigned rb, int r) {
+#pragma unroll
+    for (int pl = 0; pl < NP; ++pl) {
+      dst[pl][0] = *reinterpret_cast<const u32x4*>(smem + rb + bbase + pl * WX_XPLANE + r * WX_XROW);
+      dst[pl][1] = *reinterpret_cast<const u32x4*>(smem + rb + bbase + pl * WX_XPLANE + r * WX_XROW + 16);
+    }
+  };
+  auto read_a = [&](unsigned rb, int s) {
+#pragma unroll
+    for (int pl = 0; pl < NP; ++pl) a[s][pl] = *reinterpret_cast<const u32x4*>(smem + rb + pl * GPL + (abase ^ ((unsigned)s << 5)));
+  };
+  auto cut_s = [&](auto sc, auto hic, u32x4 (&src)[NP][2]) {
+    constexpr int pl = decltype(sc)::value >> 1, hf = decltype(sc)::value & 1, o = 4 * decltype(hic)::value;
+    const u32x4 d0 = src[pl][0], d1 = src[pl][1];
+    const unsigned d[8] = {d0[0], d0[1], d0[2], d0[3], d1[0], d1[1], d1[2], d1[3]};
+    if (hf == 1) asm volatile("" ::"v"(d[0]), "v"(d[7]));
+#pragma unroll
+    for (int j = 2 * hf; j < 2 * hf + 2; ++j) {
+      btn[0][pl][o + j] = __builtin_amdgcn_alignbit(d[j + 2], d[j + 1], 16);
+      btn[1][pl][o + j] = d[j + 2];
+      btn[2][pl][o + j] = __builtin_amdgcn_alignbit(d[j + 3], d[j + 2], 16);
+      WX_PIN(btn[0][pl][o + j]); WX_PIN(btn[1][pl][o + j]); WX_PIN(btn[2][pl][o + j]);
+    }
+  };
+  auto copy_s = [&](auto sc) {
+    constexpr int pl = decltype(sc)::value >> 1, hf = decltype(sc)::value & 1;
+#pragma unroll
+    for (int j = 2 * hf; j < 2 * hf + 2; ++j)
+#pragma unroll
+      for (int kx = 0; kx < 3; ++kx) { btn[kx][pl][j] = bt[kx][pl][4 + j]; WX_PIN(btn[kx][pl][j]); }
+  };
+
+  auto settle_bt = [&]() {
+#pragma unroll
+    for (int kx = 0; kx < 3; ++kx)
+#pragma unroll
+      for (int pl = 0; pl < NP; ++pl) {
+        bt[kx][pl] = btn[kx][pl];
+#ifdef __HIP_DEVICE_COMPILE__
+        asm volatile("" : "+v"(bt[kx][pl]));
+#endif
+      }
+#ifdef __HIP_DEVICE_COMPILE__
+    asm volatile("s_nop 1" ::: "memory");
+#endif
   };
 
   load_origin(pre[0]);
@@ -326,14 +450,23 @@
   load_origin(pre[0]);
   static_for<13>([&](auto itc) { load_step(itc, pre[0]); });
 #endif
-  read_row(0, 0);
-  static_for<2 * NP>([&](auto sc) { cut_step(sc); });
-#pragma unroll
-  for (int kx = 0; kx < 3; ++kx)
-#pragma unroll
-    for (int pl = 0; pl < NP; ++pl) b[kx][pl] = bn[kx][pl];
-
-  auto tile = [&](int i, Pre& P) {
+  if constexpr (GSP) {
+    read_prow(raw, 0, 0); read_prow(raw1, 0, 1); read_a(0, 0);
+    idxv[0] = *reinterpret_cast<const unsigned*>(smem + ibase);
+    static_for<2 * NP>([&](auto sc) { cut_s(sc, std::integral_constant<int, 0>{}, raw); });
+    static_for<2 * NP>([&](auto sc) { cut_s(sc, std::integral_constant<int, 1>{}, raw1); });
+    settle_bt();
+  } else {
+    read_row(0, 0);
+    static_for<2 * NP>([&](auto sc) { cut_step(sc); });
+#pragma unroll
+    for (int kx = 0; kx < 3; ++kx)
+#pragma unroll
+      for (int pl = 0; pl < NP; ++pl) b[kx][pl] = bn[kx][pl];
+  }
+
+  auto tile = [&](int i, Pre& P, auto parc) {
+    constexpr int PAR = decltype(parc)::value;
     const unsigned rb = (i & 1) ? LDSI : 0, wb = LDSI - rb;
     const unsigned gwb = gdst + wb, xwb = xdst + wb;
     bsum_on = i + 1 < nT;
@@ -378,18 +511,87 @@
         for (int pl = 0; pl < NP; ++pl) b[kx][pl] = bn[kx][pl];
       if (r == 4) __syncthreads();
     };
-    row(std::integral_constant<int, 0>{}); row(std::integral_constant<int, 1>{}); row(std::integral_constant<int, 2>{});
-    row(std::integral_constant<int, 3>{}); row(std::integral_constant<int, 4>{}); row(std::integral_constant<int, 5>{});
+    auto step = [&](auto rc) {
+      constexpr int r = decltype(rc)::value;
+      constexpr int npair = r == 3 ? 2 : 1;
+      constexpr int NM = 3 * NQ * npair;
+      constexpr int NPX = 9 - XPH0;
+      constexpr int NSTG = r == 1 ? 4 * 5 + NPX : (r == 2 || r == 3) ? 4 * NPX : r == 4 ? 13 : 0;
+      constexpr int NS = NSTG + 4 * NP;
+      __builtin_amdgcn_sched_barrier(0);
+      if (r < 5) {
+        read_prow(raw, rb, r + 1);
+        if (r == 1) read_a(rb, 1);
+      } else {
+        read_prow(raw, wb, 0); read_prow(raw1, wb, 1); read_a(wb, 0);
+        idxv[PAR ^ 1] = *reinterpret_cast<const unsigned*>(smem + wb + ibase);
+      }
+      __builtin_amdgcn_sched_barrier(0);
+      static_for<NM>([&](auto mc) {
+        constexpr int m = decltype(mc)::value;
+        constexpr int q = m / (3 * npair), pi = (m / 3) % npair, kx = m % 3;
+        constexpr int sp = r == 3 ? pi : r < 3 ? 0 : 1, ky = r - 1 - 2 * sp;
+        static_assert(ky >= 0 && ky < 3, "tap walk");
+        static_assert(NP == 2, "sparse products: two-plane fp16 form only");
+#ifdef __HIP_DEVICE_COMPILE__
+        if constexpr (sp == 0)
+          asm volatile("v_smfmac_f32_32x32x32_f16 %0, %1, %2, %3" : "+a"(acc[3 * ky + kx]) : "v"(a[sp][PA[q]]), "v"(bt[kx][PB[q]]), "v"(idxv[PAR]));
+        else
+          asm volatile("v_smfmac_f32_32x32x32_f16 %0, %1, %2, %3 abid:1" : "+a"(acc[3 * ky + kx]) : "v"(a[sp][PA[q]]), "v"(bt[kx][PB[q]]), "v"(idxv[PAR]));
+#endif
+        __builtin_amdgcn_sched_barrier(0);
+        constexpr int LEAD = NSTG == 0 ? 4 : 0;
+        constexpr int s0 = m < LEAD ? 0 : (m - LEAD) * NS / (NM - LEAD), s1 = m < LEAD ? 0 : (m - LEAD + 1) * NS / (NM - LEAD);
+        static_for<s1 - s0>([&](auto dc) {
+          constexpr int s = s0 + decltype(dc)::value;
+          if constexpr (s >= NSTG) {
+            constexpr int c = s - NSTG;
+            if constexpr (r == 5) {
+              if constexpr (c < 2 * NP) cut_s(std::integral_constant<int, c>{}, std::integral_constant<int, 0>{}, raw);
+              else cut_s(std::integral_constant<int, c - 2 * NP>{}, std::integral_constant<int, 1>{}, raw1);
+            } else {
+              if constexpr (c < 2 * NP) copy_s(std::integral_constant<int, c>{});
+              else cut_s(std::integral_constant<int, c - 2 * NP>{}, std::integral_constant<int, 1>{}, raw);
+            }
+          } else if constexpr (r >= 1 && r <= 3) {
+            stage_seq(std::integral_constant<int, r == 1 ? 0 : r == 2 ? 5 : 9>{}, std::integral_constant<int, s>{}, gwb, xwb, P);
+          } else {
+            if constexpr (s == 0) load_origin(P);
+            load_step(std::integral_constant<int, s>{}, P);
+          }
+        });
+        __builtin_amdgcn_sched_barrier(0);
+      });
+      settle_bt();
+      if (r == 4) __syncthreads();
+    };
+    if constexpr (GSP) {
+      step(std::integral_constant<int, 1>{}); step(std::integral_constant<int, 2>{}); step(std::integral_constant<int, 3>{});
+      step(std::integral_constant<int, 4>{}); step(std::integral_constant<int, 5>{});
+    } else {
+      row(std::integral_constant<int, 0>{}); row(std::integral_constant<int, 1>{}); row(std::integral_constant<int, 2>{});
+      row(std::integral_constant<int, 3>{}); row(std::integral_constant<int, 4>{}); row(std::integral_constant<int, 5>{});
+    }
   };
   {
     int i = 0;
 #ifdef WX_ONE_SET
-    for (; i < nT; ++i) tile(i, pre[0]);
+    for (; i < nT; ++i) {
+      if (i & 1) tile(i, pre[0], std::integral_constant<int, 1>{});
+      else tile(i, pre[0], std::integral_constant<int, 0>{});
+    }
 #else
-    for (; i + 1 < nT; i += 2) { tile(i, pre[1]); tile(i + 1, pre[0]); }
-    if (i < nT) tile(i, pre[1]);
+    for (; i + 1 < nT; i += 2) { tile(i, pre[1], std::integral_constant<int, 0>{}); tile(i + 1, pre[0], std::integral_constant<int, 1>{}); }
+    if (i < nT) tile(i, pre[1], std::integral_constant<int, 0>{});
 #endif
   }
+#ifdef __HIP_DEVICE_COMPILE__
+  if constexpr (GSP) {
+    asm volatile("s_nop 7\n\ts_nop 7\n\ts_nop 7" ::: "memory");
+#pragma unroll
+    for (int t = 0; t < 9; ++t) asm volatile("" : "+a"(acc[t]));
+  }
+#endif
   if (p.gbias && ct == 0) {
     float v = bsum;
     v += __shfl_xor(v, 1); v += __shfl_xor(v, 2);
@@ -427,19 +629,19 @@
 
 static const WgradMap* g_wx_map = nullptr;
 
-template <bool SLOPE, bool SCALE, int VEC, int NP = 3>
+template <bool SLOPE, bool SCALE, int VEC, int NP = 3, bool GSP = false>
 static int launch_wgradx_v(WgradXArgs& a, double flops, float* gw, hipStream_t s) {
   static bool attr_set = false;
   if (!attr_set) {
-    FR_HIP(hipFuncSetAttribute(reinterpret_cast<const void*>(conv_wgradx_kernel<SLOPE, SCALE, VEC, NP>),
+    FR_HIP(hipFuncSetAttribute(reinterpret_cast<const void*>(conv_wgradx_kernel<SLOPE, SCALE, VEC, NP, GSP>),
                                hipFuncAttributeMaxDynamicSharedMemorySize, NP == 2 ? 120 * 1024 : 160 * 1024));
     attr_set = true;
   }
   const int grid = a.oTiles * a.cTiles * a.nSplit;
   const double bytes = 4.0 * ((double)a.Cin * a.H * a.W + (double)a.O * a.Ho * a.Wo);
   if (prof_enabled(KC_CONV_WGRADX)) prof_before(KC_CONV_WGRADX, s);
-  const size_t lds = 2 * (size_t)NP * (WX_GPLANE + WX_XPLANE);
-  hipLaunchKernelGGL((conv_wgradx_kernel<SLOPE, SCALE, VEC, NP>), dim3(grid), dim3(256), lds, s, a);
+  const size_t lds = 2 * ((size_t)NP * ((GSP ? WX_GPLANE_S : WX_GPLANE) + WX_XPLANE) + (GSP ? WX_IPLANE : 0));
+  hipLaunchKernelGGL((conv_wgradx_kernel<SLOPE, SCALE, VEC, NP, GSP>), dim3(grid), dim3(256), lds, s, a);
   if (g_wx_map) FR_TRY(wgrad_reduce_map(a.slab, a.nSplit, 9, a.O, a.Cin, gw, *g_wx_map, s));
   else FR_TRY(wgrad_reduce(a.slab, a.nSplit, 9, a.O * a.Cin, gw, s));
   if (prof_enabled(KC_CONV_WGRADX)) prof_after(KC_CONV_WGRADX, flops, bytes, s);
@@ -454,18 +656,18 @@
   return (uintptr_t)p + bytes + slack <= (uintptr_t)base + size;
 }
 
-template <bool SLOPE, bool SCALE, int NP = 3>
+template <bool SLOPE, bool SCALE, int NP = 3, bool GSP = false>
 static int launch_wgradx(WgradXArgs& a, double flops, float* gw, hipStream_t s) {
   if (a.pad == 1 && a.W % 4 == 0 && ((uintptr_t)a.in & 15) == 0 && ((uintptr_t)a.g & 15) == 0)
-    return launch_wgradx_v<SLOPE, SCALE, 1, NP>(a, flops, gw, s);
+    return launch_wgradx_v<SLOPE, SCALE, 1, NP, GSP>(a, flops, gw, s);
   if (a.pad == 1 && readable_past_end(a.in, (size_t)a.Cin * a.H * a.W * 4, 12) && readable_past_end(a.g, (size_t)a.O * a.Ho * a.Wo * 4, 12))
-    return launch_wgradx_v<SLOPE, SCALE, 2, NP>(a, flops, gw, s);
-  return launch_wgradx_v<SLOPE, SCALE, 0, NP>(a, flops, gw, s);
+    return launch_wgradx_v<SLOPE, SCALE, 2, NP, GSP>(a, flops, gw, s);
+  return launch_wgradx_v<SLOPE, SCALE, 0, NP, GSP>(a, flops, gw, s);
 }
 
 int conv_wgradx(const float* in, int Cin, int H, int W, const float* in_slope, const float* in_scale, const float* g, int O,
                 int pad, float* gw, void* ws, size_t ws_bytes, hipStream_t s, float* gbias, const float* amax_in, const float* amax_g,
-                const WgradMap* map) {
+                const WgradMap* map, bool pooled) {
   WgradXArgs a;
   a.in = in; a.in_slope = in_slope; a.in_scale = in_scale; a.g = g; a.gbias = gbias;
   a.amax_in = amax_in; a.amax_g = amax_g;
@@ -480,6 +682,10 @@
   FR_CHECK(ws && ws_bytes >= need, "conv_wgradx: workspace too small (%zu < %zu)", ws_bytes, need);
   a.slab = (float*)(((uintptr_t)ws + 255) / 256 * 256);
   const double flops = 2.0 * O * Cin * 9 * (double)a.Ho * a.Wo;
+  if (amax_in && pooled && sparse_wgrad_on()) {
+    if (in_slope) return in_scale ? launch_wgradx<true, true, 2, true>(a, flops, gw, s) : launch_wgradx<true, false, 2, true>(a, flops, gw, s);
+    return in_scale ? launch_wgradx<false, true, 2, true>(a, flops, gw, s) : launch_wgradx<false, false, 2, true>(a, flops, gw, s);
+  }
   if (amax_in) {
     if (in_slope) return in_scale ? launch_wgradx<true, true, 2>(a, flops, gw, s) : launch_wgradx<true, false, 2>(a, flops, gw, s);
     return in_scale ? launch_wgradx<false, true, 2>(a, flops, gw, s) : launch_wgradx<false, false, 2>(a, flops, gw, s);
diff --git a/include/frcnn_hip.h b/include/frcnn_hip.h
--- a/include/frcnn_hip.h
+++ b/include/frcnn_hip.h
@@ -77,6 +77,9 @@
 int frcnn_conv2d_backward_weight(const float *in, int C, int H, int W, const float *in_slope,
                                  const float *in_scale, const float *gout, int O, int k, int pad,
                                  float *gweight, float *gbias, void *stream);
+int frcnn_conv2d_backward_weight_pooled(const float *in, int C, int H, int W, const float *in_slope,
+                                        const float *in_scale, const float *gout, int O, int k, int pad,
+                                        float *gweight, float *gbias, void *stream);
 
 int frcnn_maxpool_act_forward(const float *x, int C, int H, int W, const float *slope,
                               const float *scale, float *out, unsigned char *idx, void *stream);
```

Result: no change. 534.8, median of 6 (+0.1%).
